# lppllppl920/SAGE-SLAM

Hardware: AMD Instinct MI355X
Metric: M residuals/sec (+ LM iters/sec), 64-keyframe feature-metric BA @128x160 (higher is better)
Workload: dtype f32; 1 GPU; 64-keyframe window, 128x160x16 feature pyramids (L=4), 32-dim depth code, dense sampling N=16128, 186 links = 372 photometric + 372 geometric directed edges; parallelism=single GPU, collective=none, accepted_steps=988

## Files before the change

include/sage_ba.h:

```cpp
#ifndef SAGE_BA_H_
#define SAGE_BA_H_

#include <stddef.h>
#include <stdint.h>

#ifdef __cplusplus
extern "C" {
#endif

#define SAGE_MAX_LEVELS 8
#define SAGE_POSE_FLOATS 12

#define SAGE_OK 0
#define SAGE_E_INVALID (-1)
#define SAGE_E_UNSUPPORTED (-2)
#define SAGE_E_NOT_PSD (-3)
#define SAGE_E_STATE (-4)
#define SAGE_E_NO_OVERLAP (-5)

typedef struct SageCamera
{
  float fx, fy, cx, cy, w, h;
} SageCamera;

// ... 10 lines not shown
const char *sage_version(void);
const char *sage_error_string(int code);

typedef struct SageWorkspace SageWorkspace;
int sage_workspace_create(void *hip_stream, SageWorkspace **out);
void sage_workspace_destroy(SageWorkspace *ws);


int sage_photometric_jac_error_calculate(
    SageWorkspace *ws, float *AtA_dev, float *Atb_dev, float *error_host, float *num_inliers_host,
    const float *R10_dev, const float *t10_dev, const float *R0_dev, const float *t0_dev,
    const float *R1_dev, const float *t1_dev,
    const float *bias0_dev, const float *basis0_dev, const float *code0_dev, const float *mask1_dev,
    const int64_t *loc1d_dev, const float *homo_dev,
    const float *feat0_dev, const float *feat1_dev, const float *grad1_dev,
    float scale0, const SagePyramid *pyr, float eps, const float *weights_host,
    int N, int FS, int CS);

int sage_photometric_error_calculate(
    SageWorkspace *ws, float *error_host, float *num_inliers_host,
    const float *R10_dev, const float *t10_dev,
    const float *bias0_dev, const float *basis0_dev, const float *code0_dev, const float *mask1_dev,
    const int64_t *loc1d_dev, const float *homo_dev,
    const float *feat0_dev, const float *feat1_dev,
    float scale0, const SagePyramid *pyr, float eps, const float *weights_host,
    int N, int FS, int CS);

int sage_tracker_photo_jac_error_calculate(
    SageWorkspace *ws, int dof, float *AtA_dev, float *Atb_dev, float *error_host, float *num_inliers_host,
    const float *R_dev, const float *t_dev, const float *mask1_dev,
    const float *dpts0_dev, const float *homo_dev, const float *feat0s_dev,
    const float *feat1_dev, const float *grad1_dev,
    const SagePyramid *pyr, float scale0, float eps, const float *weights_dev, int N, int FS);

int sage_tracker_photo_error_calculate(
    SageWorkspace *ws, float *error_host, float *num_inliers_host,
    const float *R_dev, const float *t_dev, const float *mask1_dev,
    const float *dpts0_dev, const float *homo_dev, const float *feat0s_dev, const float *feat1_dev,
    const SagePyramid *pyr, float eps, const float *weights_dev, int N, int FS);

int sage_geometric_jac_error_calculate(
    SageWorkspace *ws, float *AtA_dev, float *Atb_dev, float *error_host, float *num_inliers_host,
    const float *R10_dev, const float *t10_dev, const float *R0_dev, const float *t0_dev,
    const float *R1_dev, const float *t1_dev,
    const float *bias0_dev, const float *basis0_dev, const float *code0_dev,
    const float *dpt1_dev, const float *dpt_grad1_dev, const float *basis1_dev, const float *mask1_dev,
    const int32_t *loc1d_dev, const float *homo_dev,
    float scale0, float scale1, const SageCamera *cam, float eps, float loss_param, float weight,
    int N, int CS);

int sage_geometric_error_calculate(
    SageWorkspace *ws, float *error_host, float *num_inliers_host,
    const float *R10_dev, const float *t10_dev,
    const float *bias0_dev, const float *basis0_dev, const float *code0_dev,
    const float *dpt1_dev, const float *mask1_dev, const int32_t *loc1d_dev, const float *homo_dev,
    float scale0, const SageCamera *cam, float eps, float loss_param, float weight, int N, int CS);

int sage_depth_and_grad(SageWorkspace *ws, float *dpt_dev, float *dpt_grad_dev,
                        const float *bias_dev, const float *basis_dev, const float *code_dev,
                        float scale, int H, int W, int CS);
int sage_gaussian_pyramid_with_grad(SageWorkspace *ws, float *pyr_dev, float *grad_dev,
                                    const float *feat_dev, const float *mask_dev,
                                    const SagePyramid *pyr, int FS);

int sage_bind_thread_to_device(int device);
int sage_solver_helper_cpus(int *cpus, int n);
int sage_solver_placement_moves(void);
int sage_placement_monitor(int enable);
void sage_shutdown(void);
int sage_host_threads_running(void);

void sage_se3_exp(const float *omega, const float *v, float *R, float *t);
void sage_pose_retract(const float *pose, const float *delta6, float *out);
int sage_nearest_psd(const double *M, int n, double *out);
int sage_nearest_psd_reference(const double *M, int n, double *out);
int sage_factor_block_count(int type, int CS);
int sage_factor_hessian_blocks(int type, int CS, const float *AtA_host, const float *Atb_host, int psd_mode,
                               double *G_out, double *g_out, int32_t *dims_out, int32_t *nkeys_out);
int sage_damped_solve_qr_f32(const float *A, const float *b, int n, float damp, float *x);

int sage_block_solve(const double *packed_host, int K, int nlinks, const int32_t *links, int B, double damp,
                     const double *diag_add, const double *g_add, double *delta);
long long sage_solve_lookahead_count(void);

typedef struct SageLmConfig
{
  int max_num_iters;
  float min_grad_thresh;
  float min_param_inc_thresh;
  float init_damp;
  float min_damp, max_damp;
  float damp_dec_factor;
  float damp_inc_factor;
  float jac_update_err_inc_threshold;
  int max_inner_evals;
  float no_overlap_error;
  int linearize_at_candidate;
} SageLmConfig;
void sage_lm_config_default(SageLmConfig *cfg);

typedef int (*SageTrackLinearizeFn)(void *ctx, const float *pose12, float scale, float *AtA, float *Atb, float *error);
typedef int (*SageTrackErrorFn)(void *ctx, const float *pose12, float scale, float *error);

typedef struct SageLmTraceEntry
{
  float damp, error, candidate_error;
  int accepted, relinearized;
} SageLmTraceEntry;

int sage_track_lm(const SageLmConfig *cfg, int dof, SageTrackLinearizeFn lin, SageTrackErrorFn err, void *ctx,
                  float *pose12, float *scale, float *final_error, int *iters,
                  SageLmTraceEntry *trace, int trace_cap, int *trace_len);

typedef struct SageTrackProblem
{
  SageWorkspace *ws;
  int32_t use_photo;
  const float *mask1_dev, *dpts0_dev, *homo_dev, *feat0s_dev, *feat1_dev, *grad1_dev;
  const float *weights_dev;
  SagePyramid pyr;
  float eps;
  int32_t N, FS;
  int32_t use_keypoints, NK;
  const float *kp_dpts0_dev;
  const float *kp_homo0_dev;
  const float *kp_matched_2d_dev;
  const float *kp_matched_dpts1_dev;
  const float *kp_matched_homo1_dev;
  float kp_loss_param;
  float kp_weight;
} SageTrackProblem;
int sage_track_frame(const SageLmConfig *cfg, int dof, const SageTrackProblem *prob,
                     float *pose12, float *scale, float *final_error, int *iters,
                     SageLmTraceEntry *trace, int trace_cap, int *trace_len);

typedef struct SageOverlapStats
{
  double input_area, warp_area;
  float area_ratio, inlier_ratio, average_motion;
  int32_t n_points, n_pos_depth, n_in_mask;
  int32_t n_candidates[2];
} SageOverlapStats;
int sage_track_overlap(SageWorkspace *ws, const float *R, const float *t, const float *dpts0_dev, float depth_scale,
                       const float *homo_dev, int M, const SageCamera *cam, const float *mask_dev, float eps,
                       SageOverlapStats *out);
int sage_convex_hull_area(const float *xy, int n, double *area, int *n_vertices);

typedef struct SageWindow SageWindow;

typedef struct SageKeyframeView
{
  const float *feat_pyr;
  const float *grad_pyr;
  const float *bias;
  const float *basis;
  const int64_t *loc1d;
  const float *homo;
  int32_t N;
} SageKeyframeView;

typedef struct SageWindowConfig
{
  SagePyramid pyr;
  int32_t FS, CS;
  const float *mask_dev;
  float photo_weights[SAGE_MAX_LEVELS];
// ... 105 lines not shown
                                        const float *matched_2d, const SageCamera *cam, float eps, float loss_param,
                                        float weight, int N);

enum { SAGE_LOSS_FAIR = 0, SAGE_LOSS_L2 = 1, SAGE_LOSS_HUBER = 2, SAGE_LOSS_UNBIASED = 3 };
int sage_match_geometry_jac_error_calculate(SageWorkspace *ws, float *AtA_dev, float *Atb_dev, float *error_host,
                                            const float *R10, const float *t10, const float *R0, const float *t0,
                                            const float *R1, const float *t1, const float *bias0, const float *bias1,
                                            const float *basis0, const float *basis1, const float *code0,
                                            const float *code1, const float *homo0, const float *matched_homo1,
                                            const int32_t *loc1d_0, const int32_t *matched_loc1d_1, float scale0,
                                            float scale1, float loss_param, float weight, int loss, int N, int CS);
int sage_match_geometry_error_calculate(SageWorkspace *ws, float *error_host, const float *R10, const float *t10,
                                        const float *bias0, const float *bias1, const float *basis0, const float *basis1,
                                        const float *code0, const float *code1, const float *homo0,
                                        const float *matched_homo1, const int32_t *loc1d_0,
                                        const int32_t *matched_loc1d_1, float scale0, float scale1, float loss_param,
                                        float weight, int loss, int N, int CS);
int sage_loop_mg_jac_error_calculate(SageWorkspace *ws, float *AtA_dev, float *Atb_dev, float *error_host,
                                     const float *R10, const float *t10, const float *R0, const float *t0,
                                     const float *R1, const float *t1, const float *unscaled_dpts0,
                                     const float *matched_unscaled_dpts1, const float *homo0, const float *matched_homo1,
                                     float scale0, float scale1, float loss_param, float weight, int N);
int sage_loop_mg_error_calculate(SageWorkspace *ws, float *error_host, const float *R10, const float *t10,
                                 const float *unscaled_dpts0, const float *matched_unscaled_dpts1, const float *homo0,
                                 const float *matched_homo1, float scale0, float scale1, float loss_param, float weight,
                                 int N);
int sage_tracker_match_geom_jac_error_calculate(SageWorkspace *ws, float *AtA_dev, float *Atb_dev, float *error_host,
                                                const float *R, const float *t, const float *sampled_dpts0,
                                                const float *matched_dpts1, const float *homo0,
                                                const float *matched_homo1, float scale0, float loss_param,
                                                float weight, int with_scale, int N);
int sage_tracker_match_geom_error_calculate(SageWorkspace *ws, float *error_host, const float *R, const float *t,
                                            const float *sampled_dpts0, const float *matched_dpts1, const float *homo0,
                                            const float *matched_homo1, float loss_param, float weight, int N);

int sage_cycle_match(SageWorkspace *ws, const float *desc0_dev, const float *desc1_dev, const int64_t *kp_loc1d_0,
                     int K, int C, int H, int W, float cyc_thresh, int64_t *raw_matched_loc1d_1,
                     int64_t *cyc_matched_loc1d_0, int32_t *inlier_flags, int *n_inliers_host);

int sage_sort_locations(SageWorkspace *ws, const int64_t *loc1d_dev, const float *homo_dev, int n, int H, int W,
                        int64_t *loc1d_out_dev, float *homo_out_dev, int *sorted_host);
int sage_valid_locations(SageWorkspace *ws, const float *mask_dev, const SageCamera *cam, int64_t *loc1d_dev,
                         float *homo_dev, int *n_valid_host);
int sage_shuffle_indices(int64_t seed, int64_t n, int64_t *idx_host);
int sage_sample_locations(SageWorkspace *ws, const int64_t *valid_loc1d_dev, const float *valid_homo_dev, int n_valid,
                          int64_t seed, int num_samples, int64_t *loc1d_dev, float *homo_dev, int *n_out_host);

typedef int (*SageAllReduceFn)(double *dev_buf, size_t n, void *user);
int sage_window_set_allreduce(SageWindow *w, SageAllReduceFn fn, void *user);

typedef struct SageShardPlan SageShardPlan;
int sage_shard_plan_create(int K, int nlinks, const int32_t *links, int B, int rank, int world, SageShardPlan **out);
void sage_shard_plan_destroy(SageShardPlan *p);
size_t sage_shard_sep_count(const SageShardPlan *p);
int sage_shard_num_separators(const SageShardPlan *p);
int sage_shard_num_interior(const SageShardPlan *p);
int sage_shard_keyframe_owner(const SageShardPlan *p, int kf);
int sage_shard_keyframe_is_local(const SageShardPlan *p, int kf);
int sage_shard_eliminate(SageShardPlan *p, const double *packed_local_host, double damp, const double *diag_add,
                         const double *g_add, double *sep_out);
int sage_shard_solve(SageShardPlan *p, const double *sep_reduced, double *delta);
int sage_shard_plan_create_domains(int K, int nlinks, const int32_t *links, int B, int domain, int ndomains,
                                   SageShardPlan **out);
int sage_block_solve_domains(const double *packed_host, int K, int nlinks, const int32_t *links, int B, double damp,
                             const double *diag_add, const double *g_add, int ndomains, double *delta);

int sage_window_emulate_peers(SageWindow *w, const double *rest_dev, int n_iterates);
#define SAGE_RCCL_ID_BYTES 128
int sage_rccl_unique_id(unsigned char *id128);
int sage_rccl_comm_create(const unsigned char *id128, int rank, int world, void **comm_out);
void sage_rccl_comm_destroy(void *comm);
int sage_rccl_comm_info(void *comm, int *ranks_out, int *rank_out);
int sage_window_use_rccl(SageWindow *w, void *nccl_comm);

typedef struct SageLmState
{
  double damp, error, candidate_error;
  int accepted, iters;
} SageLmState;
int sage_window_lm_step(SageWindow *w, SageLmState *st, const SageLmConfig *cfg);
int sage_window_lm_run(SageWindow *w, SageLmState *st, const SageLmConfig *cfg, int n, double *trace, int *done);
int sage_window_lm_run_timed(SageWindow *w, SageLmState *st, const SageLmConfig *cfg, int n, double *trace, int *done,
                             double *step_seconds);
int sage_window_sync_variables(SageWindow *w);

#ifdef __cplusplus
}
#endif
#endif
```

sage_slam_amd/build.py:

```python
from __future__ import annotations

import os
import subprocess
import sys
from concurrent.futures import ThreadPoolExecutor

HERE = os.path.dirname(os.path.abspath(__file__))
ROOT = os.path.dirname(HERE)
CSRC = os.path.join(HERE, "csrc")
OBJ = os.path.join(HERE, "csrc", "_obj")
LIB = os.path.join(HERE, "libsage_ba.so")
SOURCES = ["photo_kernels.hip", "geo_kernels.hip", "track_kernels.hip", "producers.hip", "keypoint_kernels.hip", "graph_kernels.hip", "solve_kernels.hip", "operators.hip", "tracker.hip", "overlap.hip", "window.hip", "window_eval.hip", "window_reduce.hip", "window_solve.hip", "window_lm.hip", "window_profile.hip", "window_build.hip", "window_terms.hip", "window_dist.hip", "window_factors.hip",
           "host_math.cpp", "block_solver.cpp", "host_threads.cpp", "shard_solve.cpp", "convex_hull.cpp"]
HEADERS = ["sage_device.h", "sage_internal.h", "damped_system.h", "host_math.h", "block_solver.h", "host_threads.h", "runtime_internal.h", "window_state.h", "finalize_bodies.h", "keypoint_batch.h", "graph_terms.h", "graph_batch.h", "term_results.h", "window_plan.h", os.path.join(ROOT, "include", "sage_ba.h")]
HIPCC = os.environ.get("HIPCC", "/opt/rocm/bin/hipcc")
HOSTCXX = os.environ.get("HOSTCXX", "/opt/rocm/lib/llvm/bin/clang++")
FLAGS = ["--offload-arch=gfx950", "-O3", "-std=c++17", "-fPIC", "-Wall", "-Wno-unused-function",
         "-I" + os.path.join(ROOT, "include"), "-I" + CSRC]


def kernel_source_sha16() -> str:
    import hashlib
    h = hashlib.sha256()
    for f in ("photo_kernels.hip", "geo_kernels.hip", "sage_device.h", "sage_internal.h"):
        with open(os.path.join(CSRC, f), "rb") as fh:
            h.update(fh.read())
    return h.hexdigest()[:16]


def _mtime(p):
    return os.path.getmtime(p) if os.path.exists(p) else 0.0


def _compile(src):
    obj = os.path.join(OBJ, os.path.splitext(src)[0] + ".o")
    deps = [os.path.join(CSRC, src)] + [h if os.path.isabs(h) else os.path.join(CSRC, h) for h in HEADERS]
    if _mtime(obj) >= max(_mtime(d) for d in deps):
        return obj, False
    if src.endswith(".hip"):
        cmd = [HIPCC] + FLAGS + ["-x", "hip", "-c", os.path.join(CSRC, src), "-o", obj]
    else:
        cmd = [HOSTCXX, "-O3", "-std=c++17", "-fPIC", "-Wall", "-I" + os.path.join(ROOT, "include"), "-I" + CSRC,
               "-c", os.path.join(CSRC, src), "-o", obj]
    subprocess.check_call(cmd)
    return obj, True


def build(force: bool = False, verbose: bool = False) -> str:
    os.makedirs(OBJ, exist_ok=True)
    if force:
        for f in os.listdir(OBJ):
            os.remove(os.path.join(OBJ, f))
    with ThreadPoolExecutor(max_workers=min(8, len(SOURCES))) as ex:
        res = list(ex.map(_compile, SOURCES))
    objs = [o for o, _ in res]
    if any(ch for _, ch in res) or not os.path.exists(LIB):
        subprocess.check_call([HIPCC, "--offload-arch=gfx950", "-shared", "-fPIC", "-o", LIB] + objs + ["-lpthread"])
        if verbose:
            print("built", LIB)
    return LIB


GLUE_SRC = os.path.join(ROOT, "integration", "compile_check", "prepass_run.cpp")
GLUE_BIN = os.path.join(ROOT, "integration", "compile_check", "_bin", "prepass_run")
REF_THIRDPARTY = "/root/reference/system/thirdparty"


def build_glue_check(verbose: bool = False):
    if not os.path.isdir(REF_THIRDPARTY):
        return GLUE_BIN if os.path.exists(GLUE_BIN) else None
    deps = [GLUE_SRC, os.path.join(ROOT, "integration", "sage_gtsam_prepass.h"), os.path.join(ROOT, "include", "sage_ba.h"),
            os.path.join(ROOT, "integration", "compile_check", "gtsam", "linear", "HessianFactor.h"),
            os.path.join(ROOT, "integration", "compile_check", "gtsam", "nonlinear", "Values.h"), LIB]
    if _mtime(GLUE_BIN) >= max(_mtime(d) for d in deps):
        return GLUE_BIN
    os.makedirs(os.path.dirname(GLUE_BIN), exist_ok=True)
    subprocess.check_call([HOSTCXX, "-std=c++17", "-O1", "-w", "-D__HIP_PLATFORM_AMD__", "-I" + os.path.join(ROOT, "include"),
                           "-I" + os.path.join(ROOT, "integration", "compile_check"), "-I" + REF_THIRDPARTY + "/eigen",
                           "-I" + REF_THIRDPARTY + "/Sophus", "-I/opt/rocm/include", GLUE_SRC, "-o", GLUE_BIN,
                           "-L" + HERE, "-lsage_ba", "-L/opt/rocm/lib", "-lamdhip64",
                           "-Wl,-rpath,$ORIGIN/../../../sage_slam_amd", "-Wl,-rpath,/opt/rocm/lib"])
    if verbose:
        print("built", GLUE_BIN)
    return GLUE_BIN


ADAPTER_BIN = os.path.join(ROOT, "integration", "compile_check", "_bin", "adapter_run")
REF_SYSTEM = "/root/reference/system"


def build_adapter_run(verbose: bool = False):
    if not os.path.isdir(REF_SYSTEM):
        return ADAPTER_BIN if os.path.exists(ADAPTER_BIN) else None
    import torch
    T = os.path.dirname(torch.__file__)
    srcs = [os.path.join(ROOT, "integration", "sage_adapter.cpp"), os.path.join(ROOT, "integration", "sage_adapter_keypoints.cpp"),
            os.path.join(ROOT, "integration", "compile_check", "adapter_run.cpp")]
# ... 31 lines not shown
```

sage_slam_amd/capi.py:

```python
from __future__ import annotations

import ctypes as C
import os
from typing import List, Optional, Sequence

import numpy as np

HERE = os.path.dirname(os.path.abspath(__file__))
LIB_PATH = os.path.join(HERE, "libsage_ba.so")
SAGE_MAX_LEVELS = 8


class SageError(RuntimeError):
    def __init__(self, code: int, where: str):
        self.code = code
        msg = lib().sage_error_string(code).decode() if _lib is not None else "?"
        super().__init__(f"{where}: {msg} (code {code})")


class SageCamera(C.Structure):
    _fields_ = [(n, C.c_float) for n in ("fx", "fy", "cx", "cy", "w", "h")]


class SagePyramid(C.Structure):
# ... 18 lines not shown
    _fields_ = [("ws", C.c_void_p), ("use_photo", C.c_int32), ("mask1_dev", C.c_void_p), ("dpts0_dev", C.c_void_p),
                ("homo_dev", C.c_void_p), ("feat0s_dev", C.c_void_p), ("feat1_dev", C.c_void_p),
                ("grad1_dev", C.c_void_p), ("weights_dev", C.c_void_p), ("pyr", SagePyramid), ("eps", C.c_float),
                ("N", C.c_int32), ("FS", C.c_int32), ("use_keypoints", C.c_int32), ("NK", C.c_int32),
                ("kp_dpts0_dev", C.c_void_p), ("kp_homo0_dev", C.c_void_p), ("kp_matched_2d_dev", C.c_void_p),
                ("kp_matched_dpts1_dev", C.c_void_p), ("kp_matched_homo1_dev", C.c_void_p),
                ("kp_loss_param", C.c_float), ("kp_weight", C.c_float)]


class SageKeyframeView(C.Structure):
    _fields_ = [("feat_pyr", C.c_void_p), ("grad_pyr", C.c_void_p), ("bias", C.c_void_p), ("basis", C.c_void_p),
                ("loc1d", C.c_void_p), ("homo", C.c_void_p), ("N", C.c_int32)]


class SageWindowConfig(C.Structure):
    _fields_ = [("pyr", SagePyramid), ("FS", C.c_int32), ("CS", C.c_int32), ("mask_dev", C.c_void_p),
                ("photo_weights", C.c_float * SAGE_MAX_LEVELS), ("geo_weight", C.c_float),
                ("geo_loss_param", C.c_float), ("eps", C.c_float), ("code_prior_weight", C.c_float),
                ("scale_prior_weight", C.c_float), ("pose_prior_weight", C.c_float),
                ("use_photo", C.c_int32), ("use_geo", C.c_int32)]


SAGE_KP_REPROJECTION, SAGE_KP_MATCH_GEOMETRY, SAGE_KP_LOOP_MG = 0, 1, 2
SAGE_HOLD_POSE, SAGE_HOLD_CODE, SAGE_HOLD_SCALE = 1, 2, 4
KP_KINDS = {"reprojection": SAGE_KP_REPROJECTION, "match_geometry": SAGE_KP_MATCH_GEOMETRY, "loop_mg": SAGE_KP_LOOP_MG}


class SageKeypointTerm(C.Structure):
    _fields_ = [("kind", C.c_int32), ("edge", C.c_int32), ("N", C.c_int32), ("loc1d_0", C.c_void_p), ("homo0", C.c_void_p),
                ("matched_2d", C.c_void_p), ("matched_loc1d_1", C.c_void_p), ("matched_homo1", C.c_void_p),
                ("loss_param", C.c_float), ("weight", C.c_float), ("loss", C.c_int32), ("unscaled_dpts0", C.c_void_p),
                ("matched_unscaled_dpts1", C.c_void_p)]


def kp_term_dim(kind, CS: int) -> int:
    kind = KP_KINDS.get(kind, kind)
    return {SAGE_KP_REPROJECTION: 13 + CS, SAGE_KP_MATCH_GEOMETRY: 14 + 2 * CS, SAGE_KP_LOOP_MG: 14}[kind]


SAGE_GRAPH_REL_POSE_SCALE, SAGE_GRAPH_REL_POSE, SAGE_GRAPH_SCALE_PRIOR = 0, 1, 2
GRAPH_KINDS = {"rel_pose_scale": SAGE_GRAPH_REL_POSE_SCALE, "rel_pose": SAGE_GRAPH_REL_POSE, "scale_prior": SAGE_GRAPH_SCALE_PRIOR}
GRAPH_TERM_DIM = 14
GRAPH_KIND_ROWS = {SAGE_GRAPH_REL_POSE_SCALE: 7, SAGE_GRAPH_REL_POSE: 6, SAGE_GRAPH_SCALE_PRIOR: 1}


class SageGraphTerm(C.Structure):
    _fields_ = [("kind", C.c_int32), ("edge", C.c_int32), ("kf", C.c_int32), ("target_pose10", C.c_float * 12),
                ("target_scale0", C.c_float), ("target_scale1", C.c_float), ("weight", C.c_float), ("rot_weight", C.c_float),
                ("scale_weight", C.c_float)]


def graph_term_struct(t) -> SageGraphTerm:
    gt = SageGraphTerm()
    gt.kind = int(GRAPH_KINDS.get(t["kind"], t["kind"]))
    gt.edge, gt.kf = int(t.get("edge", 0)), int(t.get("kf", 0))
    tp = np.asarray(t.get("target_pose10", [1, 0, 0, 0, 1, 0, 0, 0, 1, 0, 0, 0]), np.float32).reshape(12)
    for i in range(12):
        gt.target_pose10[i] = float(tp[i])
    gt.target_scale0, gt.target_scale1 = float(t.get("target_scale0", 1.0)), float(t.get("target_scale1", 1.0))
    gt.weight, gt.rot_weight, gt.scale_weight = float(t["weight"]), float(t.get("rot_weight", 1.0)), float(t.get("scale_weight", 1.0))
    return gt


ALLREDUCE_FN = C.CFUNCTYPE(C.c_int, C.c_void_p, C.c_size_t, C.c_void_p)


class SageLmState(C.Structure):
    _fields_ = [("damp", C.c_double), ("error", C.c_double), ("candidate_error", C.c_double),
                ("accepted", C.c_int), ("iters", C.c_int)]


TRACK_LIN_FN = C.CFUNCTYPE(C.c_int, C.c_void_p, C.POINTER(C.c_float), C.c_float, C.POINTER(C.c_float),
                           C.POINTER(C.c_float), C.POINTER(C.c_float))
TRACK_ERR_FN = C.CFUNCTYPE(C.c_int, C.c_void_p, C.POINTER(C.c_float), C.c_float, C.POINTER(C.c_float))

_lib = None

SYMBOLS = [
    "sage_camera_pyramid", "sage_version", "sage_error_string", "sage_workspace_create", "sage_workspace_destroy",
    "sage_photometric_jac_error_calculate", "sage_photometric_error_calculate",
    "sage_tracker_photo_jac_error_calculate", "sage_tracker_photo_error_calculate",
    "sage_geometric_jac_error_calculate", "sage_geometric_error_calculate", "sage_depth_and_grad",
    "sage_gaussian_pyramid_with_grad", "sage_se3_exp", "sage_pose_retract", "sage_nearest_psd", "sage_nearest_psd_reference", "sage_factor_block_count", "sage_factor_hessian_blocks",
    "sage_damped_solve_qr_f32", "sage_block_solve", "sage_solve_lookahead_count", "sage_lm_config_default", "sage_track_lm", "sage_track_frame", "sage_track_overlap", "sage_convex_hull_area",
    "sage_window_create", "sage_window_destroy", "sage_window_add_keyframe", "sage_window_add_link", "sage_window_add_keypoint_link", "sage_window_hold", "sage_window_set_link_geo_loss",
    "sage_window_set_shard", "sage_window_finalize", "sage_window_num_keyframes", "sage_window_num_links",
    "sage_window_block_size", "sage_window_solver_block_size", "sage_window_packed_count", "sage_window_packed_dev",
    "sage_window_residuals_per_linearize", "sage_window_bytes_per_linearize", "sage_window_linearize",
    "sage_window_error", "sage_window_tune_runs", "sage_window_set_runs", "sage_window_error_dev", "sage_window_solve", "sage_window_total_error",
    "sage_window_accept", "sage_window_reset", "sage_window_get_keyframe", "sage_window_set_keyframe", "sage_window_get_delta",
    "sage_window_get_edge", "sage_window_add_keypoint_term", "sage_window_num_keypoint_terms", "sage_window_get_keypoint_term", "sage_window_add_graph_term", "sage_window_num_graph_terms", "sage_window_get_graph_term", "sage_window_prepass", "sage_window_factor", "sage_window_factor_error", "sage_window_prepare_factors", "sage_factor_psd", "sage_factor_cut_blocks", "sage_window_set_profiling", "sage_window_get_kernel_time", "sage_window_get_phase_time", "sage_window_lm_step", "sage_window_lm_run", "sage_window_lm_run_timed", "sage_window_sync_variables", "sage_window_set_allreduce", "sage_shard_plan_create", "sage_shard_plan_create_domains", "sage_block_solve_domains", "sage_shard_plan_destroy", "sage_shard_sep_count", "sage_shard_num_separators", "sage_shard_num_interior", "sage_shard_keyframe_owner", "sage_shard_keyframe_is_local", "sage_shard_eliminate", "sage_shard_solve", "sage_rccl_unique_id", "sage_rccl_comm_create", "sage_rccl_comm_destroy", "sage_rccl_comm_info", "sage_window_use_rccl", "sage_window_emulate_peers", "sage_sort_locations", "sage_bind_thread_to_device", "sage_solver_helper_cpus", "sage_solver_placement_moves", "sage_placement_monitor", "sage_shutdown", "sage_host_threads_running",
    "sage_valid_locations", "sage_shuffle_indices", "sage_sample_locations",
    "sage_reprojection_jac_error_calculate", "sage_reprojection_error_calculate",
    "sage_tracker_reproj_jac_error_calculate", "sage_tracker_reproj_error_calculate",
    "sage_match_geometry_jac_error_calculate", "sage_match_geometry_error_calculate",
    "sage_loop_mg_jac_error_calculate", "sage_loop_mg_error_calculate",
    "sage_tracker_match_geom_jac_error_calculate", "sage_tracker_match_geom_error_calculate", "sage_cycle_match",
]


def lib():
    global _lib
    if _lib is None:
        LIB_PATH = os.environ.get("SAGE_BA_LIB", globals()["LIB_PATH"])
        if not os.path.exists(LIB_PATH):
            raise ImportError(f"{LIB_PATH} is missing: run `python -m sage_slam_amd.build` "
                              "(the HIP engine has no fallback path)")
        import torch
        L = C.CDLL(LIB_PATH)
        L.sage_version.restype = C.c_char_p
        L.sage_error_string.restype = C.c_char_p
        L.sage_window_packed_count.restype = C.c_size_t
        L.sage_shutdown.restype = None
        L.sage_window_packed_dev.restype = C.c_void_p
        L.sage_window_error_dev.restype = C.c_void_p
        L.sage_window_residuals_per_linearize.restype = C.c_double
        L.sage_window_bytes_per_linearize.restype = C.c_double
        for name in ("sage_window_packed_count", "sage_window_packed_dev", "sage_window_error_dev",
                     "sage_window_residuals_per_linearize", "sage_window_bytes_per_linearize",
                     "sage_window_num_keyframes", "sage_window_num_links", "sage_window_block_size",
                     "sage_window_solver_block_size"):
            getattr(L, name).argtypes = [C.c_void_p]
        _lib = L
    return _lib


def _chk(code: int, where: str):
    if code != 0:
        raise SageError(code, where)


def _f32(a) -> np.ndarray:
    return np.ascontiguousarray(a, dtype=np.float32)


def _fp(a: np.ndarray):
    return a.ctypes.data_as(C.POINTER(C.c_float))


def dptr(t) -> C.c_void_p:
    if t is None:
        return C.c_void_p(0)
    assert t.is_contiguous(), "device buffers handed to the C ABI must be contiguous"
    return C.c_void_p(t.data_ptr())


def make_pyramid(cam, levels: int) -> SagePyramid:
    base = SageCamera(*[float(v) for v in (cam.fx, cam.fy, cam.cx, cam.cy, cam.w, cam.h)])
    out = SagePyramid()
    _chk(lib().sage_camera_pyramid(C.byref(base), levels, C.byref(out)), "sage_camera_pyramid")
    return out


def se3_exp(omega, v):
    omega = _f32(omega); v = _f32(v)
    R = np.zeros(9, np.float32); t = np.zeros(3, np.float32)
    lib().sage_se3_exp(_fp(omega), _fp(v), _fp(R), _fp(t))
    return R.reshape(3, 3), t


def pose_retract(pose12, delta6):
    pose12 = _f32(pose12).reshape(12); delta6 = _f32(delta6)
    out = np.zeros(12, np.float32)
    lib().sage_pose_retract(_fp(pose12), _fp(delta6), _fp(out))
    return out


def nearest_psd(M):
    M = np.ascontiguousarray(M, dtype=np.float64)
    out = np.zeros_like(M)
    _chk(lib().sage_nearest_psd(M.ctypes.data_as(C.POINTER(C.c_double)), M.shape[0],
                                out.ctypes.data_as(C.POINTER(C.c_double))), "sage_nearest_psd")
    return out


def nearest_psd_reference(M):
    M = np.ascontiguousarray(M, np.float64)
    out = np.zeros_like(M)
    _chk(lib().sage_nearest_psd_reference(M.ctypes.data_as(C.POINTER(C.c_double)), M.shape[0],
                                          out.ctypes.data_as(C.POINTER(C.c_double))), "sage_nearest_psd_reference")
    return out


def factor_hessian_blocks(type_: int, CS: int, AtA, Atb, psd_mode: int = 1):
    L = lib()
    A = _f32(AtA); b = _f32(Atb)
    n = L.sage_factor_block_count(type_, CS)
    if n < 0:
        raise SageError(n, "sage_factor_block_count")
    G = np.zeros(n, np.float64); g = np.zeros(b.size, np.float64)
    dims = (C.c_int32 * 6)(); nk = C.c_int32()
    _chk(L.sage_factor_hessian_blocks(type_, CS, _fp(A), _fp(b), psd_mode, G.ctypes.data_as(C.POINTER(C.c_double)),
                                      g.ctypes.data_as(C.POINTER(C.c_double)), dims, C.byref(nk)),
         "sage_factor_hessian_blocks")
    dims = [int(dims[i]) for i in range(nk.value)]
    blocks, o = {}, 0
    for i in range(nk.value):
        for j in range(i, nk.value):
            blocks[(i, j)] = G[o:o + dims[i] * dims[j]].reshape(dims[i], dims[j]); o += dims[i] * dims[j]
    offs = np.concatenate([[0], np.cumsum(dims)])
    return blocks, [g[offs[i]:offs[i + 1]] for i in range(nk.value)], dims


def damped_solve_qr_f32(A, b, damp):
    A = _f32(A); b = _f32(b)
    x = np.zeros(b.shape[0], np.float32)
    _chk(lib().sage_damped_solve_qr_f32(_fp(A), _fp(b), b.shape[0], C.c_float(damp), _fp(x)), "sage_damped_solve_qr_f32")
    return x


def block_solve(packed, K, links, B, damp, diag_add=None, g_add=None):
    packed = np.ascontiguousarray(packed, dtype=np.float64)
    lk = np.ascontiguousarray(np.asarray(links, dtype=np.int32).reshape(-1))
    delta = np.zeros(K * B, np.float64)
    dp = lambda a: None if a is None else np.ascontiguousarray(a, np.float64).ctypes.data_as(C.POINTER(C.c_double))
    da = None if diag_add is None else np.ascontiguousarray(diag_add, np.float64)
    ga = None if g_add is None else np.ascontiguousarray(g_add, np.float64)
    _chk(lib().sage_block_solve(packed.ctypes.data_as(C.POINTER(C.c_double)), K, len(lk) // 2, lk.ctypes.data_as(C.POINTER(C.c_int32)), B,
                                C.c_double(damp), dp(da), dp(ga), delta.ctypes.data_as(C.POINTER(C.c_double))),
         "sage_block_solve")
    return delta


def solve_lookahead_count() -> int:
    f = lib().sage_solve_lookahead_count
    f.restype = C.c_longlong
    return int(f())


def block_solve_domains(packed, K, links, B, damp, ndomains, diag_add=None, g_add=None):
    p = np.ascontiguousarray(packed, np.float64)
    lk = np.ascontiguousarray(np.asarray(links, np.int32).reshape(-1))
    out = np.zeros(K * B, np.float64)
    dp = lambda a: None if a is None else np.ascontiguousarray(a, np.float64).ctypes.data_as(C.POINTER(C.c_double))
    da = None if diag_add is None else np.ascontiguousarray(diag_add, np.float64)
    ga = None if g_add is None else np.ascontiguousarray(g_add, np.float64)
    _chk(lib().sage_block_solve_domains(p.ctypes.data_as(C.POINTER(C.c_double)), K, len(links),
                                        lk.ctypes.data_as(C.POINTER(C.c_int32)), B, C.c_double(damp), dp(da), dp(ga),
                                        ndomains, out.ctypes.data_as(C.POINTER(C.c_double))), "sage_block_solve_domains")
    return out


def lm_config_default() -> SageLmConfig:
    cfg = SageLmConfig()
    lib().sage_lm_config_default(C.byref(cfg))
    return cfg


def pack_pose(R, t) -> np.ndarray:
    return np.concatenate([_f32(R).reshape(9), _f32(t).reshape(3)])


def track_lm(cfg: SageLmConfig, dof: int, lin_fn, err_fn, pose12, scale: float, trace_cap: int = 256):
    def _lin(ctx, p, s, AtA, Atb, err):
        A, b, e = lin_fn(np.ctypeslib.as_array(p, (12,)).copy(), float(s))
        A = _f32(A).reshape(-1); b = _f32(b).reshape(-1)
        for i in range(dof * dof):
            AtA[i] = A[i]
        for i in range(dof):
            Atb[i] = b[i]
        err[0] = e
        return 0

    def _err(ctx, p, s, err):
        err[0] = err_fn(np.ctypeslib.as_array(p, (12,)).copy(), float(s))
        return 0

    pose = _f32(pose12).reshape(12).copy()
    sc = C.c_float(scale)
    fe = C.c_float(0); it = C.c_int(0); tl = C.c_int(0)
    trace = (SageLmTraceEntry * trace_cap)()
    cb1, cb2 = TRACK_LIN_FN(_lin), TRACK_ERR_FN(_err)
    _chk(lib().sage_track_lm(C.byref(cfg), dof, cb1, cb2, None, _fp(pose), C.byref(sc), C.byref(fe), C.byref(it),
                             trace, trace_cap, C.byref(tl)), "sage_track_lm")
    tr = [dict(damp=trace[i].damp, error=trace[i].error, candidate_error=trace[i].candidate_error,
               accepted=trace[i].accepted, relinearized=trace[i].relinearized) for i in range(tl.value)]
    return pose, sc.value, fe.value, it.value, tr


def track_frame(cfg: SageLmConfig, dof: int, prob: "SageTrackProblem", pose12, scale: float, trace_cap: int = 256):
    L = lib()
    p = _f32(pose12).copy()
    sc = C.c_float(scale); fe = C.c_float(); it = C.c_int(); tl = C.c_int()
    tr = (SageLmTraceEntry * trace_cap)()
    rc = L.sage_track_frame(C.byref(cfg), dof, C.byref(prob), _fp(p), C.byref(sc), C.byref(fe), C.byref(it), tr,
                            trace_cap, C.byref(tl))
    trace = [dict(damp=tr[i].damp, error=tr[i].error, candidate_error=tr[i].candidate_error,
                  accepted=tr[i].accepted, relinearized=tr[i].relinearized) for i in range(tl.value)]
    return rc, p, sc.value, fe.value, it.value, trace


class SageOverlapStats(C.Structure):
    _fields_ = [("input_area", C.c_double), ("warp_area", C.c_double), ("area_ratio", C.c_float),
                ("inlier_ratio", C.c_float), ("average_motion", C.c_float), ("n_points", C.c_int32),
                ("n_pos_depth", C.c_int32), ("n_in_mask", C.c_int32), ("n_candidates", C.c_int32 * 2)]


def track_overlap_raw(ws_handle, R, t, dpts0_ptr, depth_scale, homo_ptr, M, cam_ptr, mask_ptr, eps, out_ptr) -> int:
    f = lib().sage_track_overlap
    f.argtypes = [C.c_void_p, C.c_void_p, C.c_void_p, C.c_void_p, C.c_float, C.c_void_p, C.c_int, C.c_void_p, C.c_void_p,
                  C.c_float, C.c_void_p]
    return int(f(ws_handle, R, t, dpts0_ptr, depth_scale, homo_ptr, int(M), cam_ptr, mask_ptr, eps, out_ptr))


# ... 320 lines not shown
        return out

    def packed_tensor(self):
        return _tensor_from_ptr(lib().sage_window_packed_dev(self.h), self.packed_count)

    def error_tensor(self):
        return _tensor_from_ptr(lib().sage_window_error_dev(self.h), 4)

    def linearize(self):
        _chk(lib().sage_window_linearize(self.h), "sage_window_linearize")

    def error(self, which=1):
        _chk(lib().sage_window_error(self.h, which), "sage_window_error")

    def tune_runs(self):
        tpb, rule = C.c_int(0), C.c_int(0)
        ms_rule, ms_best = C.c_float(0), C.c_float(0)
        _chk(lib().sage_window_tune_runs(self.h, C.byref(tpb), C.byref(rule), C.byref(ms_rule), C.byref(ms_best)),
             "sage_window_tune_runs")
        return dict(tpb=tpb.value, tpb_rule=rule.value, ms_rule=ms_rule.value, ms_best=ms_best.value)

    def set_runs(self, tpb):
        _chk(lib().sage_window_set_runs(self.h, int(tpb)), "sage_window_set_runs")

    def solve(self, damp, want_norm=True):
        if not want_norm:
            _chk(lib().sage_window_solve(self.h, C.c_double(damp), None), "sage_window_solve")
            return None
        sn = C.c_double()
        _chk(lib().sage_window_solve(self.h, C.c_double(damp), C.byref(sn)), "sage_window_solve")
        return sn.value

    def total_error(self, from_linearize: bool):
        e = C.c_double()
        _chk(lib().sage_window_total_error(self.h, int(from_linearize), C.byref(e)), "sage_window_total_error")
        return e.value

    def accept(self):
        _chk(lib().sage_window_accept(self.h), "sage_window_accept")

    def reset(self):
        _chk(lib().sage_window_reset(self.h), "sage_window_reset")

    def set_allreduce(self, dist_module, group=None):
        tensors = {}
        for t in (self.packed_tensor(), self.error_tensor()):
            tensors[(t.data_ptr(), t.numel())] = t

        def hook(ptr, n, _user):
            try:
                t = tensors.get((ptr, n))
                if t is None:
                    t = tensors[(ptr, n)] = _tensor_from_ptr(ptr, n)
                dist_module.all_reduce(t, group=group)
                return 0
            except Exception:
                import traceback
                traceback.print_exc()
                return 1

        self._allreduce_cb = ALLREDUCE_FN(hook)
        _chk(lib().sage_window_set_allreduce(self.h, self._allreduce_cb, None), "sage_window_set_allreduce")

    def sync_variables(self):
        _chk(lib().sage_window_sync_variables(self.h), "sage_window_sync_variables")

    def use_rccl(self, comm):
        _chk(lib().sage_window_use_rccl(self.h, C.c_void_p(comm)), "sage_window_use_rccl")

    def emulate_peers(self, rest):
        if rest is None:
            self._emu_rest = None
            _chk(lib().sage_window_emulate_peers(self.h, None, 0), "sage_window_emulate_peers")
            return
        assert rest.is_cuda and rest.dim() == 2 and rest.shape[1] == self.packed_count and rest.is_contiguous()
        self._emu_rest = rest
        _chk(lib().sage_window_emulate_peers(self.h, C.c_void_p(rest.data_ptr()), int(rest.shape[0])),
             "sage_window_emulate_peers")

    def lm_step(self, state: SageLmState, cfg: SageLmConfig):
        _chk(lib().sage_window_lm_step(self.h, C.byref(state), C.byref(cfg)), "sage_window_lm_step")
        return state

    def lm_run(self, state: SageLmState, cfg: SageLmConfig, n: int):
        tr = np.zeros((n, 4), np.float64)
        done = C.c_int()
        _chk(lib().sage_window_lm_run(self.h, C.byref(state), C.byref(cfg), n, tr.ctypes.data_as(C.POINTER(C.c_double)),
                                      C.byref(done)), "sage_window_lm_run")
        return tr[:done.value]

    def lm_run_timed(self, state: SageLmState, cfg: SageLmConfig, n: int):
        tr = np.zeros((n, 4), np.float64); sec = np.zeros(n, np.float64)
        done = C.c_int()
        _chk(lib().sage_window_lm_run_timed(self.h, C.byref(state), C.byref(cfg), n, tr.ctypes.data_as(C.POINTER(C.c_double)),
                                            C.byref(done), sec.ctypes.data_as(C.POINTER(C.c_double))), "sage_window_lm_run_timed")
        return tr[:done.value], sec[:done.value]

    def delta(self):
        d = np.zeros(self.K * self.B, np.float64)
        _chk(lib().sage_window_get_delta(self.h, d.ctypes.data_as(C.POINTER(C.c_double))), "sage_window_get_delta")
        return d

    def get_keyframe(self, k):
        pose = np.zeros(12, np.float32); code = np.zeros(self.win.CS, np.float32); s = C.c_float()
        _chk(lib().sage_window_get_keyframe(self.h, k, _fp(pose), _fp(code), C.byref(s)), "sage_window_get_keyframe")
        return pose, code, s.value

    def set_keyframe(self, k, pose12, code, scale):
        pose12 = _f32(pose12); code = _f32(code)
        _chk(lib().sage_window_set_keyframe(self.h, k, _fp(pose12), _fp(code), C.c_float(scale)),
             "sage_window_set_keyframe")

    def get_edge(self, type_, e):
        D = 13 + self.win.CS if type_ == 0 else 14 + 2 * self.win.CS
        A = np.zeros((D, D), np.float32); b = np.zeros(D, np.float32)
        err = C.c_float(); nin = C.c_float()
        _chk(lib().sage_window_get_edge(self.h, type_, e, _fp(A), _fp(b), C.byref(err), C.byref(nin)),
             "sage_window_get_edge")
        return dict(AtA=A, Atb=b, error=err.value, num_inliers=nin.value)

    def prepass(self, poses12, codes, scales, jacobians: bool = True) -> bool:
        P = _f32(np.asarray(poses12).reshape(-1)); Cd = _f32(np.asarray(codes).reshape(-1)); S = _f32(np.asarray(scales).reshape(-1))
        K = self.K
        assert P.size == K * 12 and Cd.size == K * self.win.CS and S.size == K
        rec = C.c_int32()
        _chk(lib().sage_window_prepass(self.h, _fp(P), _fp(Cd), _fp(S), int(jacobians), C.byref(rec)), "sage_window_prepass")
        return bool(rec.value)

    def factor(self, type_, e, psd_mode: int = 1):
        L = lib(); CS = self.win.CS
        n = L.sage_factor_block_count(type_, CS)
        D = 13 + CS if type_ == 0 else 14 + 2 * CS
        G = np.zeros(n, np.float64); g = np.zeros(D, np.float64); f = C.c_double()
        dims = (C.c_int32 * 6)(); nk = C.c_int32()
        _chk(L.sage_window_factor(self.h, type_, e, psd_mode, G.ctypes.data_as(C.POINTER(C.c_double)),
                                  g.ctypes.data_as(C.POINTER(C.c_double)), C.byref(f), dims, C.byref(nk)), "sage_window_factor")
        dims = [int(dims[i]) for i in range(nk.value)]
        blocks, o = {}, 0
        for i in range(nk.value):
            for j in range(i, nk.value):
                blocks[(i, j)] = G[o:o + dims[i] * dims[j]].reshape(dims[i], dims[j]); o += dims[i] * dims[j]
        offs = np.concatenate([[0], np.cumsum(dims)])
        return blocks, [g[offs[i]:offs[i + 1]] for i in range(nk.value)], f.value, dims

    def prepare_factors(self, psd_mode: int = 1, n_threads: int = 0):
        _chk(lib().sage_window_prepare_factors(self.h, psd_mode, n_threads), "sage_window_prepare_factors")

    def factor_error(self, type_, e) -> float:
        v = C.c_double()
        _chk(lib().sage_window_factor_error(self.h, type_, e, C.byref(v)), "sage_window_factor_error")
        return v.value

    def set_profiling(self, on):
        _chk(lib().sage_window_set_profiling(self.h, int(on)), "sage_window_set_profiling")

    def kernel_time(self, which: int):
        ms = C.c_double(); n = C.c_int()
        _chk(lib().sage_window_get_kernel_time(self.h, which, C.byref(ms), C.byref(n)), "sage_window_get_kernel_time")
        return ms.value, n.value

    def phase_time(self):
        ms = (C.c_double * 4)(); n = C.c_int()
        _chk(lib().sage_window_get_phase_time(self.h, ms, C.byref(n)), "sage_window_get_phase_time")
        return dict(zip(("linearize", "allreduce", "solve", "error_pass"), (float(v) for v in ms))), n.value

    def packed_host(self):
# ... 366 lines not shown
```

sage_slam_amd/csrc/block_solver.cpp:

```cpp
#include <algorithm>
#include <atomic>
#include <chrono>
#include <cmath>
#include <cstdio>
#include <cstdlib>
#include <cstring>
#include <sched.h>
#include <thread>
#include <vector>

#include "block_solver.h"
#include "damped_system.h"
#include "host_math.h"
#include "sage_ba.h"

namespace sage
{
namespace
{
typedef double v8d __attribute__((vector_size(64), aligned(8)));

#define SAGE_LOADU(dst, p) __builtin_memcpy(&(dst), (p), sizeof(v8d))
#define SAGE_STOREU(p, v) __builtin_memcpy((p), &(v), sizeof(v8d))

// ... 1498 lines not shown
  {
    const int rc = block_chol_range(E0, T, X, y, 0, K);
    return rc ? rc : block_back_range(E0, T, X, y, 0, K);
  }
  const int sep0 = E0.n1 + E0.n2;
  BlockEnvelope E = E0;
  const bool arrow = block_plan_has_arrow_rows(E0);
  SepJob job;
  SepPool *pool = nullptr;
  if (arrow)
  {
    job.E = &E; job.T = T; job.X = X; job.y = y;
    sep_job_build(job);
    job.t_start = mono_seconds();
    E.progress = job.progress;
    pool = pool_engage(job);
  }
  BlockEnvelope::RowPipe pipes[2];
  E.pipe = pipes;
  static const bool no_sep_pre = sage::env_flag("SAGE_SOLVE_NO_SEP_PRE");
  E.sep_pre = !arrow && !no_sep_pre;
  CholHelper *h = helper_engage(E, T, X, y);
  const bool piped = lookahead_engage(1, E, T, X, y, 0, E.n1);
  const bool dbg = debug_timing();
  double tp[6] = {0, 0, 0, 0, 0, 0};
  auto lap = [&](int k) {
    if (dbg)
      tp[k] = mono_seconds();
  };
  lap(0);
  int rc = block_chol_range(E, T, X, y, 0, E.n1, piped ? RowRole::chain : RowRole::whole);
  if (piped)
    lookahead_release(1);
  lap(1);
  const bool helper_has_it = h && helper_claimed(h);
  const int rc2 = helper_has_it ? helper_join_factor(h) : rc == 0 ? block_chol_range(E, T, X, y, E.n1, sep0) : 0;
  lap(2);
  if (rc == 0)
    rc = rc2;
  if (arrow)
    rc = arrow_separator(job, rc, tp[2]);
  else if (rc == 0)
    rc = block_chol_range(E, T, X, y, sep0, K);
  if (rc == 0)
    block_back_range(E, T, X, y, sep0, K);
  if (arrow)
  {
    arrow_back_substitute(job, E, rc);
    if (pool)
      pool_release(pool);
  }
  lap(3);
  if (helper_has_it)
    helper_go_back(h, rc == 0);
  if (rc == 0)
  {
    block_back_range(E, T, X, y, 0, E.n1);
    if (!helper_has_it)
      block_back_range(E, T, X, y, E.n1, sep0);
  }
  lap(4);
  if (helper_has_it)
    helper_join_back(h);
  lap(5);
  if (dbg)
    fprintf(stderr, "[sage block chol] us: first half %.0f (+wait for the %s %.0f) separator %.0f%s back-subst %.0f (+wait %.0f)\n",
            1e6 * (tp[1] - tp[0]), helper_has_it ? "helper" : "second half, same thread", 1e6 * (tp[2] - tp[1]),
            1e6 * (tp[3] - tp[2]), arrow ? (pool ? " (arrow rows, worker pool)" : " (arrow rows, no pool)") : "",
            1e6 * (tp[4] - tp[3]), 1e6 * (tp[5] - tp[4]));
  if (h)
    helper_release(h);
  return rc;
}

BlockEnvelope envelope_of(const BlockPlan &plan, int Bp)
{
  BlockEnvelope env;
  env.K = (int)plan.row_first.size(); env.Bp = Bp; env.n1 = plan.n1; env.n2 = plan.n2;
  env.row_first = plan.row_first.data(); env.row_off = plan.row_off.data();
  env.a_first = plan.a_first.data(); env.a_cnt = plan.a_cnt.data(); env.a_off = plan.a_off.data();
  env.col_ptr = plan.col_ptr.data(); env.col_rows = plan.col_rows.data();
  return env;
}
}

extern "C" long long sage_solve_lookahead_count(void) { return sage::g_lookahead_count.load(); }

extern "C" int sage_block_solve(const double *packed, int K, int nlinks, const int32_t *links, int B, double damp,
                                const double *diag_add, const double *g_add, double *delta)
{
  if (!packed || K < 1 || B < 1 || nlinks < 0 || (nlinks > 0 && !links) || !delta)
    return SAGE_E_INVALID;
  const int Bp = sage::padded_block(B);
  if (Bp == 0)
    return SAGE_E_UNSUPPORTED;
  const int BB = B * B, BBp = Bp * Bp;
  const double *diag = packed;
  const double *lnk = diag + (size_t)K * BB;
  const double *g = lnk + (size_t)nlinks * BB;
  std::vector<std::pair<int, int>> lk(nlinks);
  for (int l = 0; l < nlinks; ++l)
    lk[l] = {links[2 * l], links[2 * l + 1]};
  sage::BlockPlan bp;
  int rcp = sage::plan_blocks(K, lk, !sage::env_flag("SAGE_SOLVE_NO_SPLIT"), bp);
  if (rcp == SAGE_E_UNSUPPORTED)
  {
    std::sort(lk.begin(), lk.end());
    lk.erase(std::unique(lk.begin(), lk.end()), lk.end());
    rcp = sage::plan_blocks(K, lk, !sage::env_flag("SAGE_SOLVE_NO_SPLIT"), bp);
  }
  if (rcp != SAGE_OK)
    return rcp;
  const int nblk = bp.nblk;
  std::vector<double> T((size_t)nblk * BBp, 0.0), X((size_t)K * BBp), y((size_t)K * Bp, 0.0);
  for (int q = 0; q < K; ++q)
  {
    const int k = bp.perm[q];
    double *D = T.data() + (size_t)bp.index(q, q) * BBp;
    for (int r = 0; r < Bp; ++r)
      for (int c = 0; c < Bp; ++c)
        D[sage::stored_slot(r, c, Bp)] =
            (r < B && c < B) ? sage::damped_diag_elem(diag + (size_t)k * BB, B, r, c, diag_add ? diag_add[k * B + r] : 0.0, damp)
                             : sage::damped_pad_elem(r, c, damp);
    for (int r = 0; r < B; ++r)
      y[(size_t)q * Bp + r] = sage::damped_rhs_elem(g[(size_t)k * B + r], g_add ? g_add[k * B + r] : 0.0);
  }
  for (int l = 0; l < nlinks; ++l)
  {
    const int a = links[2 * l], b = links[2 * l + 1];
    const int qi = std::max(bp.pos[a], bp.pos[b]), qj = std::min(bp.pos[a], bp.pos[b]);
    double *D = T.data() + (size_t)bp.index(qi, qj) * BBp;
    const bool row_is_a = bp.perm[qi] == a;
    for (int r = 0; r < B; ++r)
      for (int c = 0; c < B; ++c)
        D[sage::stored_slot(r, c, Bp)] += lnk[(size_t)l * BB + sage::link_elem(row_is_a, r, c, B)];
  }
  static const bool dbg = sage::env_flag("SAGE_DEBUG_TIMING");
  const auto t0 = std::chrono::steady_clock::now();
  sage::BlockEnvelope env = sage::envelope_of(bp, Bp);
  int rcf;
  {
    sage::SolveLease lease;
    if (bp.n1 > 0)
      env.no_lookahead = sage::block_chol_arm(sage::block_plan_has_arrow_rows(env), sage::block_plan_long_arrow_chains(env));
    rcf = sage::block_chol_solve_tr(env, T.data(), X.data(), y.data());
  }
  if (dbg)
    fprintf(stderr, "[sage block_solve] fixed-block Cholesky + substitution %.3f ms\n",
            std::chrono::duration<double, std::milli>(std::chrono::steady_clock::now() - t0).count());
  if (rcf != 0)
    return SAGE_E_NOT_PSD;
  for (int k = 0; k < K; ++k)
    std::memcpy(delta + (size_t)k * B, y.data() + (size_t)bp.pos[k] * Bp, sizeof(double) * B);
  return SAGE_OK;
}
```

sage_slam_amd/csrc/block_solver.h:

```cpp
#pragma once
#include <stdint.h>

#include <algorithm>
#include <atomic>
#include <utility>
#include <vector>

#include "host_threads.h"

namespace sage
{
inline int padded_block(int B) { return B < 1 ? 0 : B <= 8 ? 8 : B <= 24 ? 24 : B <= 40 ? 40 : 0; }

struct BlockEnvelope
{
  int K = 0, Bp = 0;
  const int32_t *row_first = nullptr, *row_off = nullptr;
  const int32_t *a_first = nullptr, *a_cnt = nullptr, *a_off = nullptr;
  int n1 = 0, n2 = 0;
  const volatile unsigned *ready = nullptr;
  unsigned epoch = 0;
  const uint8_t *fill = nullptr;
  bool no_lookahead = false;
  std::atomic<int> *progress = nullptr;
  const int32_t *col_ptr = nullptr, *col_rows = nullptr;
  int bs_skip_from = 0x7fffffff;
  struct RowPipe
  {
    alignas(64) std::atomic<int> early{0};
    alignas(64) std::atomic<int> late{0};
    alignas(64) std::atomic<int> pre{0};
  };
  RowPipe *pipe = nullptr;
  bool sep_pre = false;

  struct Range
  {
    int lo, hi;
  };
  Range a_range(int i) const
  {
    const int a = a_cnt ? a_first[i] : 0;
    return {a, a + (a_cnt ? a_cnt[i] : 0)};
  }
  Range b_range(int i) const { return {row_first[i], i}; }
  bool has(int i, int j) const
  {
    const Range a = a_range(i);
    return (j >= row_first[i] && j <= i) || (j >= a.lo && j < a.hi);
  }
  size_t index(int i, int j) const
  {
    return (size_t)(j < row_first[i] ? a_off[i] + j - a_first[i] : row_off[i] + j - row_first[i]);
  }
  double *block(double *T, int i, int j) const { return T + index(i, j) * (size_t)(Bp * Bp); }
  Range sep_range(int srow, int half) const
  {
    if (half == 0)
      return a_range(srow);
    const int sep0 = n1 + n2;
    return {std::min((int)row_first[srow], sep0), sep0};
  }
};
int block_chol_solve_tr(const BlockEnvelope &env, double *T, double *X, double *y);
int block_chol_partial(const BlockEnvelope &env, double *T, double *X, double *y, int nI);
int block_chol_partial_back(const BlockEnvelope &env, double *T, double *X, double *y, int nI);
int block_plan_long_arrow_chains(const BlockEnvelope &env);
bool block_plan_has_arrow_rows(const BlockEnvelope &env);

struct BlockPlan
{
  std::vector<int32_t> perm, pos, row_first, row_off, a_first, a_cnt, a_off, blk_row, blk_col, blk_src;
  std::vector<int32_t> col_ptr, col_rows;
  int nblk = 0, n1 = 0, n2 = 0;
  int index(int i, int j) const
  {
    return j < row_first[i] ? a_off[i] + j - a_first[i] : row_off[i] + j - row_first[i];
  }
};
int plan_blocks(int K, const std::vector<std::pair<int, int>> &links, bool may_split, BlockPlan &out);
BlockEnvelope envelope_of(const BlockPlan &plan, int Bp);
}
```

sage_slam_amd/csrc/runtime_internal.h:

```cpp
#pragma once

#include <hip/hip_runtime.h>

#include <algorithm>
#include <atomic>
#include <cctype>
#include <sched.h>
#include <chrono>
#include <cmath>
#include <cstdlib>
#include <cstdio>
#include <cstring>
#include <thread>
#include <vector>

#include <dlfcn.h>
#if __has_include(<rccl/rccl.h>)
#include <rccl/rccl.h>
#else
extern "C"
{
  typedef struct ncclComm *ncclComm_t;
  typedef struct
  {
    char internal[128];
  } ncclUniqueId;
  typedef enum { ncclSuccess = 0 } ncclResult_t;
  typedef enum { ncclSum = 0 } ncclRedOp_t;
  typedef enum { ncclDouble = 8 } ncclDataType_t;
}
#endif

#include "host_math.h"
#include "host_threads.h"
#include "sage_ba.h"
#include "sage_internal.h"
#include "keypoint_batch.h"
#include "graph_batch.h"
#include "window_plan.h"

using namespace sage;

#define SAGE_HIP(expr)                \
  do                                  \
  {                                   \
    hipError_t _e = (expr);           \
    if (_e != hipSuccess)             \
      return (int)_e;                 \
  } while (0)

namespace sage_rt
{

struct DevBuf
{
  void *p = nullptr;
  size_t cap = 0;
  DevBuf() = default;
  DevBuf(const DevBuf &) = delete;
  DevBuf &operator=(const DevBuf &) = delete;
  DevBuf(DevBuf &&o) noexcept { swap(o); }
  DevBuf &operator=(DevBuf &&o) noexcept
  {
    DevBuf(std::move(o)).swap(*this);
    return *this;
  }
  ~DevBuf() { release(); }
  void swap(DevBuf &o) noexcept
  {
    std::swap(p, o.p);
    std::swap(cap, o.cap);
  }
  int reserve(size_t bytes)
  {
    if (bytes <= cap)
      return 0;
    release();
    hipError_t e = hipMalloc(&p, bytes);
    if (e != hipSuccess)
    {
      p = nullptr;
      return (int)e;
    }
    cap = bytes;
    return 0;
  }
  void release()
  {
    if (p)
      (void)hipFree(p);
    p = nullptr;
    cap = 0;
  }
  template <class T>
  T *as() const { return reinterpret_cast<T *>(p); }
};

inline int pick_tiles_per_block(long long total_tiles)
{
  if (total_tiles >= 8192)
    return 4;
  if (total_tiles >= 4096)
    return 2;
  return 1;
}

struct WorkList
{
  std::vector<WorkItem> work;
  std::vector<int32_t> edge_first, edge_tiles;
  std::vector<int32_t> rec_first, rec_count;
  int tiles_per_block = 1;
  int flush = 1;
  int n_records = 0;
  void build(const std::vector<int> &N, int tpb_override = 0, const std::vector<int> *order = nullptr, int flush_ = 0)
  {
    long long total = 0;
    for (int n : N)
      total += (n + kTile - 1) / kTile;
// ... 48 lines not shown
static inline bool supported(int CS, int FS)
{
  return (CS == 16 || CS == 32) && (FS == 16 || FS == 32);
}

namespace sage
{
struct AdjEntry
{
  int32_t type;
  int32_t edge;
  int32_t role;
};

struct LinkEdges
{
  int32_t e_ab, e_ba;
};

struct AssembleParams
{
  const float *AtA_p, *Atb_p, *stats_p;
  const float *AtA_g, *Atb_g, *stats_g;
  const double *wide_p, *wide_g;
  const int32_t *adj_start;
  const AdjEntry *adj;
  const LinkEdges *links;
  double *packed;
  double *tail_mirror;
  int K, nlinks, CS, n_edges_p, n_edges_g;
  int split;
  const int32_t *blocks;
  const int32_t *link_terms_start;
  const AdjEntry *link_terms;
  TermResults terms;
};

struct ErrorTotalsSide
{
  const int32_t *edge_first, *edge_tiles;
  const float *partials;
  float *stats;
  float fallback, scale;
  int n_edges;
  int stride, err_off, cnt_off;
};

}

#include "window_state.h"

struct SageWindow
{
  SageWindowConfig cfg;
  hipStream_t stream = nullptr;
  bool finalized = false;
  int rank = 0, world = 1;
  int K = 0, B = 0, VS = 0;
  std::vector<SageKeyframeView> views;
  HostVars hv;
  std::vector<float> link_geo_loss;
  std::vector<std::pair<int, int>> links;
  std::vector<char> link_dense;
  std::vector<uint8_t> hold;
  sage::plan::SolverRows rows;
  std::vector<int> local_links;
  std::vector<int> owned_edges;
  std::vector<int> local_edges;
  int n_edges = 0;
  DevBuf vars[2];
  DevBuf sorted_loc, sorted_homo;
  std::vector<std::pair<const int64_t *, const float *>> user_samples;
  std::vector<int> user_n;
  DevBuf dpt, dgrad, depth_items[2];
  int n_depth = 0;
  int dpt_set = -1;
  bool dgrad_valid = false;
  DevBuf geo_px;
  bool merge_ok = false;
  DevBuf pk;
  DevBuf f0s;
  DenseSide dense[2];
  PhotoRecordPlan photo_rec;
  std::vector<int> Nedge;
  int tpb_heur = 1;
  DevBuf adj_start, adj, link_edges, packed, errbuf;
  TotalsMirror mirror;
  WindowDist dist;
  std::vector<double> host_packed;
  std::vector<double> delta;
  sage::DeviceSolver *solver = nullptr;
  bool cand_pending = false;
  double residuals_per_lin = 0, bytes_per_lin = 0;
  bool have_lin = false;
  uint64_t vars_epoch = 1, lin_epoch = 0;
  bool spec_err_valid = false;
  double spec_error = 0.0;
  DevBuf packed_save;
  TermSide terms;
  struct FactorCache
  {
    bool lin = false, err = false;
    std::vector<float> pose, code, scale;
    struct Side
    {
      std::vector<float> A, b, s;
      std::vector<double> C;
    } side[2];
    int psd_mode = -1;
  } fc;
  WindowProfiler prof;

  bool kernels_mirror_totals() const { return world == 1 && !dist.allreduce && mirror.h; }
};


template <class T>
static int upload(DevBuf &b, const std::vector<T> &v, hipStream_t s)
{
  int rc = b.reserve(std::max<size_t>(v.size(), 1) * sizeof(T));
  if (rc)
    return rc;
  if (!v.empty())
    SAGE_HIP(hipMemcpyAsync(b.p, v.data(), v.size() * sizeof(T), hipMemcpyHostToDevice, s));
  return 0;
}
int window_upload_vars(SageWindow *w, int set);
int window_local_edge(const SageWindow *w, int global_edge);
bool window_owns_edge(const SageWindow *w, int global_edge);
bool window_has_holds(const SageWindow *w);
std::vector<int32_t> window_link_pairs(const SageWindow *w);
struct FinalizeState
{
  bool domain_solve = false;
  std::vector<char> needed;
  std::vector<size_t> f0s_off;
  std::vector<size_t> px_off;
  std::vector<int> Nedge;
  std::vector<std::vector<AdjEntry>> adjv;
  std::vector<LinkEdges> le;
  std::vector<char> link_terms;
  double residuals = 0, bytes = 0;
};
int finalize_terms(SageWindow *w, FinalizeState &fs);
int window_launch_terms(SageWindow *w, int set, bool jac);
int window_linearize_set(SageWindow *w, int set, double *dst = nullptr, bool local_blocks = false, bool merge = false);
int window_error_pass(SageWindow *w, int which, bool speculate_gradients);
int window_collective(SageWindow *w, double *buf, size_t n);
int window_allreduce(SageWindow *w, double *buf, size_t n, int iterate);
int window_allreduce_into(SageWindow *w, const double *send, double *recv, size_t n, int iterate);
int window_mirror_totals(SageWindow *w, bool with_err, const double *system = nullptr);
bool window_wait_error_totals(SageWindow *w);
bool window_wait_reduced_totals(SageWindow *w);
int window_wait_mirror(SageWindow *w, bool *not_psd);
double mirrored_error(const SageWindow *w, int at, int set);
int window_total_error(SageWindow *w, int from_linearize, double *err, bool stream_idle);
int window_copy_floats(SageWindow *w, const float *src, float *dst, int n);
void window_add_to_double(SageWindow *w, double *p, double v);
double window_prior_error(const SageWindow *w, int set, bool owned_only = false);
int window_sync_candidate(SageWindow *w, bool stream_idle = false);
int window_schur_solve(SageWindow *w, double damp, double *lin_error);
void prof_attach(SageWindow *w, int which, LaunchCommon &lc);
void window_phase_mark(SageWindow *w, int which);
```

sage_slam_amd/csrc/solve_kernels.hip:

```cpp
#include <algorithm>
#include <atomic>
#include <chrono>
#include <cstdio>
#include <cstring>
#include <memory>
#include <vector>

#include "block_solver.h"
#include "damped_system.h"
#include "host_math.h"
#include "sage_device.h"
#include "sage_internal.h"
#include "window_plan.h"

namespace sage
{

struct SolvePlan
{
  int K, B, Bs, Bp, nblk, nlinks;
  const int32_t *row_first;
  const int32_t *row_off;
  const int32_t *blk_row, *blk_col, *blk_src;
  const int32_t *perm, *pos;
  const int32_t *hold;
  const int32_t *to_block, *to_solver;
};

struct SolveResult
{
  double step_norm2;
  int status;
  unsigned go;
};
static size_t result_vars_offset() { return sizeof(SolveResult); }
static size_t result_delta_offset(int K, int VS) { return (sizeof(SolveResult) + (size_t)K * VS * sizeof(float) + 15) / 16 * 16; }

constexpr int kScatterWorkgroups = 32;

__global__ __launch_bounds__(256) void solve_scatter_kernel(const SolvePlan P, const double *__restrict__ packed,
                                                            const float *__restrict__ vars0, int VS, int CS,
                                                            const SolvePriors pri, double damp,
                                                            double *__restrict__ L, double *__restrict__ y,
                                                            const int32_t *__restrict__ order, unsigned *flags,
                                                            unsigned epoch)
{
  const int tid = threadIdx.x;
  const int B = P.B, Bs = P.Bs, Bp = P.Bp, BB = B * B;
  __shared__ double s_dadd[64], s_gadd[64];
  __shared__ int s_row[64];
  if (tid < Bs)
    s_row[tid] = P.to_block[tid];
  __syncthreads();
  for (int it = blockIdx.x; it < P.nblk; it += gridDim.x)
  {
    const int b = order[it];
    const int i = P.blk_row[b], j = P.blk_col[b], srcf = P.blk_src[b];
    const int src = srcf < 0 ? -1 : (srcf & 0x3fffffff);
    const bool row_is_a = srcf >= 0 && (srcf & 0x40000000);
    if (src < 0 && i != j)
      continue;
    const int kf = P.perm[i];
    const int hold_r = P.hold ? P.hold[kf] : 0, hold_c = P.hold ? P.hold[P.perm[j]] : 0;
    const double *diag = packed + (size_t)kf * BB;
    const double *lnk = packed + (size_t)P.K * BB + (size_t)(src < 0 ? 0 : src) * BB;
    const double *g = packed + (size_t)P.K * BB + (size_t)P.nlinks * BB + (size_t)kf * B;
    double *out = L + (size_t)b * Bp * Bp;
    if (i == j)
    {
      const float *var = vars0 + (size_t)kf * VS;
      if (tid < Bs)
      {
        double da, ga;
        prior_row(pri, kf, s_row[tid], CS, var, var[12], var + 13, da, ga, hold_r);
        s_dadd[tid] = da;
        s_gadd[tid] = ga;
      }
      __syncthreads();
    }
    for (int o = tid; o < Bp * Bp; o += blockDim.x)
    {
      const int c = o / Bp, r = o - c * Bp;
      double v = 0.0;
      const bool in = r < Bs && c < Bs;
      const bool held = in && solver_elem_held(hold_r, hold_c, s_row, r, c, CS);
      if (i == j)
        v = in ? (held ? held_diag_elem(r, c) : solver_diag_elem(diag, B, s_row, r, c, s_dadd[r], damp))
               : damped_pad_elem(r, c, damp);
      else if (in && !held)
        v = lnk[solver_link_elem(row_is_a, s_row, r, c, B)];
      out[o] = v;
    }
    if (i == j)
      for (int r = tid; r < Bp; r += blockDim.x)
        y[(size_t)i * Bp + r] =
            (r < Bs && !(hold_r && row_held(hold_r, s_row[r], CS))) ? damped_rhs_elem(g[s_row[r]], s_gadd[r]) : 0.0;
    __syncthreads();
    if (tid == 0)
    {
      __threadfence_system();
      *reinterpret_cast<volatile unsigned *>(flags + b) = epoch;
    }
  }
}

__global__ __launch_bounds__(1024) void solve_retract_kernel(const double *__restrict__ x, int K, int B, int Bp, int CS,
                                                            int VS, const int32_t *__restrict__ pos,
                                                            const int32_t *__restrict__ hold,
                                                            const int32_t *__restrict__ to_solver,
                                                            const float *__restrict__ vars0,
                                                            float *__restrict__ vars1, float *__restrict__ h_vars,
                                                            double *__restrict__ h_delta, SolveResult *h_res,
                                                            unsigned epoch)
{
  const int tid = threadIdx.x;
  const volatile unsigned *go = &h_res->go;
  __shared__ int s_go;
  if (tid == 0)
  {
    const unsigned long long t0 = wall_clock64();
    unsigned v;
    bool timed_out = false;
    for (;;)
    {
      v = *go;
      const unsigned d = ((v & 0x7fffffffu) - epoch) & 0x7fffffffu;
      if (d == 0u)
        break;
      if (d < 0x40000000u && (v & 0x7fffffffu) != 0u)
      {
        v = 0x80000000u;
        break;
      }
      __builtin_amdgcn_s_sleep(4);
      if (wall_clock64() - t0 > 200000000ull)
      {
        v = 0x80000000u;
// ... 26 lines not shown
      h_vars[(size_t)k * VS + slot] = v;
    }
  }
  for (int k = tid; k < K; k += blockDim.x)
  {
    const double *xk = x + (size_t)pos[k] * Bp;
    const float *v0 = vars0 + (size_t)k * VS;
    float *o = vars1 + (size_t)k * VS;
    if (hold && (hold[k] & kHoldPose))
      for (int i = 0; i < 12; ++i)
        o[i] = v0[i];
    else
    {
      float d6[6];
      for (int i = 0; i < 6; ++i)
        d6[i] = (float)xk[to_solver[i]];
      pose_retract(v0, d6, o);
    }
    for (int i = 0; i < 12; ++i)
      h_vars[(size_t)k * VS + i] = o[i];
  }
  __shared__ double s_n[16];
  for (int off = 32; off > 0; off >>= 1)
    nrm += __shfl_down(nrm, off);
  if ((tid & 63) == 0)
    s_n[tid >> 6] = nrm;
  __syncthreads();
  if (tid == 0)
  {
    double tot = 0.0;
    for (int w = 0; w < (int)(blockDim.x >> 6); ++w)
      tot += s_n[w];
    h_res->step_norm2 = tot;
  }
}

struct DeviceSolver
{
  int K = 0, B = 0, Bs = 0, Bp = 0, nblk = 0, nlinks = 0, VS = 0;
  void *d_int = nullptr;
  void *d_hold = nullptr;
  void *h_pinned = nullptr;
  void *h_T = nullptr;
  double *h_y = nullptr;
  unsigned *h_flags = nullptr;
  unsigned epoch = 0, go_epoch = 0;
  SolvePlan plan{};
  const int32_t *d_order = nullptr;
  std::vector<double> h_X;
  BlockPlan host_plan;
  std::vector<uint8_t> h_fill;

  DeviceSolver() = default;
  DeviceSolver(const DeviceSolver &) = delete;
  DeviceSolver &operator=(const DeviceSolver &) = delete;
  ~DeviceSolver()
  {
    if (d_int)
      (void)hipFree(d_int);
    if (d_hold)
      (void)hipFree(d_hold);
    if (h_pinned)
      (void)hipHostFree(h_pinned);
    if (h_T)
      (void)hipHostFree(h_T);
  }
  SolveResult *result() const { return reinterpret_cast<SolveResult *>(h_pinned); }
  float *host_vars() const { return reinterpret_cast<float *>(reinterpret_cast<char *>(h_pinned) + result_vars_offset()); }
  double *host_delta() const { return reinterpret_cast<double *>(reinterpret_cast<char *>(h_pinned) + result_delta_offset(K, VS)); }
};

int solver_create(DeviceSolver **out, int K, const plan::SolverRows &rows, int VS,
                  const std::vector<std::pair<int, int>> &links, hipStream_t stream)
{
  *out = nullptr;
  const int B = rows.B, Bs = rows.Bs;
  const int Bp = sage::padded_block(Bs);
  if (Bp == 0 || K < 1)
    return SAGE_E_UNSUPPORTED;
  BlockPlan bp;
  const int rcp = plan_blocks(K, links, !sage::env_flag("SAGE_SOLVE_NO_SPLIT"), bp);
  if (rcp != SAGE_OK)
    return rcp;
  const int n1 = bp.n1, n2 = bp.n2, nblk = bp.nblk;
  const std::vector<int32_t> &perm = bp.perm, &pos = bp.pos, &row_first = bp.row_first, &row_off = bp.row_off,
                             &a_cnt = bp.a_cnt, &a_off = bp.a_off, &blk_row = bp.blk_row, &blk_col = bp.blk_col,
                             &blk_src = bp.blk_src;
  std::unique_ptr<DeviceSolver> S(new DeviceSolver);
  S->K = K; S->B = B; S->Bs = Bs; S->Bp = Bp; S->nblk = nblk; S->nlinks = (int)links.size(); S->VS = VS;
  std::vector<int32_t> all;
  auto put = [&](const std::vector<int32_t> &v) {
    const size_t off = all.size();
    all.insert(all.end(), v.begin(), v.end());
    while (all.size() % 4)
      all.push_back(0);
    return off;
  };
  const size_t o_rf = put(row_first), o_ro = put(row_off), o_br = put(blk_row), o_bc = put(blk_col),
               o_bs = put(blk_src), o_pm = put(perm), o_ps = put(pos);
  std::vector<int32_t> order;
  auto push_row = [&](int i) {
    for (int q = 0; q < a_cnt[i]; ++q)
      order.push_back(a_off[i] + q);
    for (int q = 0; q <= i - row_first[i]; ++q)
      order.push_back(row_off[i] + q);
  };
  if (n1 > 0)
  {
    for (int t = 0; t < std::max(n1, n2); ++t)
    {
      if (t < n1)
        push_row(t);
      if (t < n2)
        push_row(n1 + t);
    }
    for (int i = n1 + n2; i < K; ++i)
      push_row(i);
  }
  else
    for (int i = 0; i < K; ++i)
      push_row(i);
  const size_t o_ord = put(order);
  const size_t o_tb = put(rows.to_block), o_ts = put(rows.to_solver);
  if (hipMalloc(&S->d_int, all.size() * sizeof(int32_t)) != hipSuccess)
    return (int)hipErrorOutOfMemory;
  if (hipMemcpyAsync(S->d_int, all.data(), all.size() * sizeof(int32_t), hipMemcpyHostToDevice, stream) != hipSuccess)
    return (int)hipErrorUnknown;
  if (hipStreamSynchronize(stream) != hipSuccess)
    return (int)hipErrorUnknown;
  const size_t ty_doubles = (size_t)nblk * Bp * Bp + (size_t)K * Bp;
  if (hipHostMalloc(&S->h_T, ty_doubles * sizeof(double) + (size_t)nblk * sizeof(unsigned), hipHostMallocDefault) !=
      hipSuccess)
    return (int)hipErrorOutOfMemory;
  S->h_y = reinterpret_cast<double *>(S->h_T) + (size_t)nblk * Bp * Bp;
  S->h_flags = reinterpret_cast<unsigned *>(reinterpret_cast<double *>(S->h_T) + ty_doubles);
  std::memset(S->h_flags, 0, (size_t)nblk * sizeof(unsigned));
  S->h_X.assign((size_t)K * Bp * Bp, 0.0);
  const size_t h_bytes = result_delta_offset(K, VS) + (size_t)K * B * sizeof(double);
  if (hipHostMalloc(&S->h_pinned, h_bytes, hipHostMallocDefault) != hipSuccess)
    return (int)hipErrorOutOfMemory;
  std::memset(S->h_pinned, 0, h_bytes);
  const int32_t *base = reinterpret_cast<const int32_t *>(S->d_int);
  SolvePlan &P = S->plan;
  P.K = K; P.B = B; P.Bs = Bs; P.Bp = Bp; P.nblk = nblk; P.nlinks = (int)links.size();
  P.row_first = base + o_rf; P.row_off = base + o_ro;
  P.blk_row = base + o_br; P.blk_col = base + o_bc; P.blk_src = base + o_bs; P.perm = base + o_pm; P.pos = base + o_ps;
  P.to_block = base + o_tb; P.to_solver = base + o_ts;
  S->d_order = base + o_ord;
  S->h_fill.assign((size_t)nblk, 0);
  for (int b = 0; b < nblk; ++b)
    S->h_fill[b] = (blk_src[b] < 0 && blk_row[b] != blk_col[b]) ? 1 : 0;
  S->host_plan = std::move(bp);
  *out = S.release();
  return SAGE_OK;
}

void solver_destroy(DeviceSolver *S) { delete S; }

int solver_set_holds(DeviceSolver *S, const std::vector<uint8_t> &hold, hipStream_t stream)
{
  if ((int)hold.size() != S->K)
    return SAGE_E_INVALID;
  const std::vector<int32_t> masks(hold.begin(), hold.end());
  if (!S->d_hold && hipMalloc(&S->d_hold, masks.size() * sizeof(int32_t)) != hipSuccess)
    return (int)hipErrorOutOfMemory;
  if (hipMemcpyAsync(S->d_hold, masks.data(), masks.size() * sizeof(int32_t), hipMemcpyHostToDevice, stream) != hipSuccess ||
      hipStreamSynchronize(stream) != hipSuccess)
    return (int)hipErrorUnknown;
  S->plan.hold = reinterpret_cast<const int32_t *>(S->d_hold);
  return SAGE_OK;
}

int solver_run(DeviceSolver *S, hipStream_t stream, const double *packed_dev, const float *vars0, float *vars1,
               int CS, double damp, const SolvePriors &pri)
{
  static const bool dbgt = sage::env_flag("SAGE_DEBUG_TIMING");
  hipError_t eh;
  SolveLease lease;
  BlockEnvelope env = envelope_of(S->host_plan, S->Bp);
  if (env.n1 > 0)
    env.no_lookahead = block_chol_arm(block_plan_has_arrow_rows(env), block_plan_long_arrow_chains(env));
  S->epoch += 1;
  if (S->epoch == 0)
    S->epoch = 1;
  hipLaunchKernelGGL(solve_scatter_kernel, dim3(std::min(kScatterWorkgroups, S->nblk)), dim3(256), 0, stream, S->plan,
                     packed_dev, vars0, S->VS, CS, pri, damp, reinterpret_cast<double *>(S->h_T), S->h_y, S->d_order,
                     S->h_flags, S->epoch);
  if ((eh = hipGetLastError()) != hipSuccess)
    return (int)eh;
  volatile unsigned *go = &S->result()->go;
  S->go_epoch = (S->go_epoch + 1) & 0x7fffffffu;
  if (S->go_epoch == 0)
    S->go_epoch = 1;
  hipLaunchKernelGGL(solve_retract_kernel, dim3(1), dim3(1024), 0, stream, S->h_y, S->K, S->B, S->Bp, CS, S->VS,
                     S->plan.pos, S->plan.hold, S->plan.to_solver, vars0, vars1, S->host_vars(), S->host_delta(),
                     S->result(), S->go_epoch);
  if ((eh = hipGetLastError()) != hipSuccess)
    return (int)eh;
  struct GoGuard
  {
    volatile unsigned *go;
    unsigned word;
    ~GoGuard()
    {
      std::atomic_thread_fence(std::memory_order_release);
      *go = word;
    }
  } guard{go, S->go_epoch | 0x80000000u};
  const auto t1 = std::chrono::steady_clock::now();
  env.ready = S->h_flags; env.epoch = S->epoch;
  env.fill = S->h_fill.data();
  const int bad = block_chol_solve_tr(env, reinterpret_cast<double *>(S->h_T), S->h_X.data(), S->h_y);
  const auto t2 = std::chrono::steady_clock::now();
  if (dbgt)
    fprintf(stderr, "[sage hybrid solve] wait for the system + host cholesky %.3f ms\n",
            std::chrono::duration<double, std::milli>(t2 - t1).count());
  if (bad == -2)
    return SAGE_E_STATE;
  if (bad)
    return SAGE_E_NOT_PSD;
  guard.word = S->go_epoch;
  return SAGE_OK;
}

const float *solver_host_vars(const DeviceSolver *S) { return S->host_vars(); }
const double *solver_host_delta(const DeviceSolver *S) { return S->host_delta(); }
double solver_host_step_norm2(const DeviceSolver *S) { return S->result()->step_norm2; }
int solver_host_status(const DeviceSolver *S) { return S->result()->status; }

}
```

sage_slam_amd/csrc/window_build.hip:

```cpp
#include "runtime_internal.h"
#include "window_plan.h"

static std::atomic<int> g_live_windows{0};

extern "C" int sage_window_create(const SageWindowConfig *cfg, void *hip_stream, SageWindow **out)
{
  if (!cfg || !out || !cfg->mask_dev)
    return SAGE_E_INVALID;
  if (!supported(cfg->CS, cfg->FS) || cfg->pyr.levels < 1 || cfg->pyr.levels > SAGE_MAX_LEVELS)
    return SAGE_E_UNSUPPORTED;
  int ndev = 0;
  SAGE_HIP(hipGetDeviceCount(&ndev));
  if (ndev < 1)
    return (int)hipErrorNoDevice;
  SageWindow *w = new SageWindow();
  w->cfg = *cfg;
  w->stream = reinterpret_cast<hipStream_t>(hip_stream);
  w->B = 7 + cfg->CS;
  w->VS = ((13 + cfg->CS + 3) / 4) * 4;
  *out = w;
  g_live_windows.fetch_add(1, std::memory_order_acq_rel);
  return SAGE_OK;
}

// ... 16 lines not shown
}

extern "C" int sage_window_add_keyframe(SageWindow *w, const SageKeyframeView *v, const float *pose12,
                                        const float *code, float scale)
{
  if (!w || !v || !pose12 || !code || w->finalized)
    return SAGE_E_INVALID;
  if (!v->feat_pyr || !v->grad_pyr || !v->bias || !v->basis || !v->loc1d || !v->homo || v->N < 0)
    return SAGE_E_INVALID;
  w->views.push_back(*v);
  for (int s = 0; s < 2; ++s)
  {
    w->hv.pose[s].insert(w->hv.pose[s].end(), pose12, pose12 + 12);
    w->hv.code[s].insert(w->hv.code[s].end(), code, code + w->cfg.CS);
    w->hv.scale[s].push_back(scale);
  }
  w->hv.pose_init.insert(w->hv.pose_init.end(), pose12, pose12 + 12);
  w->hv.code_added.insert(w->hv.code_added.end(), code, code + w->cfg.CS);
  w->hv.scale_init.push_back(scale);
  return w->K++;
}

static int add_link(SageWindow *w, int a, int b, char dense)
{
  if (a == b || a < 0 || b < 0 || a >= w->K || b >= w->K)
    return SAGE_E_INVALID;
  w->links.emplace_back(std::min(a, b), std::max(a, b));
  w->link_geo_loss.push_back(0.f);
  w->link_dense.push_back(dense);
  return (int)w->links.size() - 1;
}

extern "C" int sage_window_add_link(SageWindow *w, int a, int b) { return !w || w->finalized ? SAGE_E_INVALID : add_link(w, a, b, 1); }
extern "C" int sage_window_add_keypoint_link(SageWindow *w, int a, int b)
{
  return !w ? SAGE_E_INVALID : (w->finalized ? SAGE_E_STATE : add_link(w, a, b, 0));
}

extern "C" int sage_window_hold(SageWindow *w, int kf, int what)
{
  if (!w)
    return SAGE_E_INVALID;
  if (w->finalized)
    return SAGE_E_STATE;
  if (kf < 0 || kf >= w->K || what < 0 || what > (SAGE_HOLD_POSE | SAGE_HOLD_CODE | SAGE_HOLD_SCALE))
    return SAGE_E_INVALID;
  w->hold.resize(w->K, 0);
  w->hold[kf] = (uint8_t)what;
  return SAGE_OK;
}

extern "C" int sage_window_set_link_geo_loss(SageWindow *w, int link, float loss_param)
{
  if (!w || w->finalized || link < 0 || link >= (int)w->links.size() || !(loss_param >= 0.f))
    return w && w->finalized ? SAGE_E_STATE : SAGE_E_INVALID;
  w->link_geo_loss[link] = loss_param;
  return SAGE_OK;
}

static int photo_flush_for_runs(int tpb)
{
  if (const char *e = getenv("SAGE_PHOTO_FLUSH"))
    return std::max(0, atoi(e));
  return plan::record_cadence(tpb);
}

static int upload_work_list(DenseSide &sd, const WorkList &wl, hipStream_t s)
{
  int rc;
  sd.n_work = (int)wl.work.size();
  sd.tpb = wl.tiles_per_block;
  if ((rc = upload(sd.work, wl.work, s)) || (rc = upload(sd.first, wl.edge_first, s)) || (rc = upload(sd.tiles, wl.edge_tiles, s)))
    return rc;
  return SAGE_OK;
}

static void window_invalidate_plan_results(SageWindow *w)
{
  w->have_lin = false;
  w->spec_err_valid = false;
  w->dpt_set = -1;
}

static int window_plan_photo_runs(SageWindow *w, int tpb, int flush)
{
  WorkList wp;
  wp.build(w->Nedge, tpb, nullptr, flush);
  int rc;
  w->photo_rec.flush = wp.flush;
  w->photo_rec.n = wp.n_records;
  DenseSide &ph = w->dense[kPhoto];
  if ((rc = upload_work_list(ph, wp, w->stream)) || (rc = upload(w->photo_rec.first, wp.rec_first, w->stream)) ||
      (rc = upload(w->photo_rec.count, wp.rec_count, w->stream)))
    return rc;
  SAGE_HIP(hipStreamSynchronize(w->stream));
  return ph.part.reserve(std::max<size_t>(1, std::max(ph.n_work, w->photo_rec.n)) * photo_partial_floats(w->cfg.CS) * sizeof(float));
}

static std::vector<int> edge_tiles(const std::vector<int> &Nedge)
{
  std::vector<int> tiles;
  for (int n : Nedge)
    tiles.push_back((n + kTile - 1) / kTile);
  return tiles;
}

static int image_pixels(const SageWindow *w) { return (int)w->cfg.pyr.cam[0].h * (int)w->cfg.pyr.cam[0].w; }

static int finalize_variables(SageWindow *w)
{
  const int K = w->K, HW = image_pixels(w);
  int rc;
  for (int s = 0; s < 2; ++s)
  {
    if ((rc = w->vars[s].reserve((size_t)K * w->VS * sizeof(float))))
      return rc;
    if ((rc = window_upload_vars(w, s)))
      return rc;
  }
  if ((rc = w->dpt.reserve((size_t)K * HW * sizeof(float))) || (rc = w->dgrad.reserve((size_t)K * 2 * HW * sizeof(float))))
    return rc;
  return SAGE_OK;
}

static int finalize_ownership(SageWindow *w, FinalizeState &fs)
{
  const int K = w->K, HW = image_pixels(w);
  int rc;
  const bool by_link = sage::env_flag("SAGE_SHARD_BY_LINK") || fs.domain_solve;
  plan::Ownership own = plan::owned_edges((int)w->links.size(), w->rank, w->world, by_link);
  w->owned_edges = std::move(own.edges);
  w->local_links = std::move(own.links);
  w->local_edges = plan::dense_edges(w->owned_edges, w->link_dense);
  fs.needed.assign(K, 0);
  for (int ge : w->local_edges)
    fs.needed[w->links[ge / 2].first] = fs.needed[w->links[ge / 2].second] = 1;
  w->n_depth = 0;
  for (int k = 0; k < K; ++k)
    w->n_depth += fs.needed[k];
  for (int s = 0; s < 2; ++s)
  {
    std::vector<DepthItem> items;
    for (int k = 0; k < K; ++k)
    {
      if (!fs.needed[k])
        continue;
      const float *vp = w->vars[s].as<float>() + (size_t)k * w->VS;
      items.push_back(DepthItem{w->views[k].bias, w->views[k].basis, vp + 13, vp + 12,
                                w->dpt.as<float>() + (size_t)k * HW, w->dgrad.as<float>() + (size_t)k * 2 * HW});
    }
    if ((rc = upload(w->depth_items[s], items, w->stream)))
      return rc;
    SAGE_HIP(hipStreamSynchronize(w->stream));
  }
  return SAGE_OK;
}

static int finalize_pyramids(SageWindow *w)
{
  const SageWindowConfig &c = w->cfg;
  const int FS = c.FS, K = w->K;
  int rc;
  const size_t plane_f = (size_t)FS * c.pyr.P;
  if ((rc = w->pk.reserve((size_t)K * 3 * plane_f * sizeof(float))))
    return rc;
  float lvl_scale[SAGE_MAX_LEVELS] = {};
  for (int l = 0; l < c.pyr.levels; ++l)
  {
    if (!(c.photo_weights[l] >= 0.f))
      return SAGE_E_INVALID;
    lvl_scale[l] = std::sqrt(c.photo_weights[l]);
  }
  for (int k = 0; k < K; ++k)
  {
    float *base = w->pk.as<float>() + (size_t)k * 3 * plane_f;
    SAGE_HIP(launch_repack_groups(w->stream, base, w->views[k].feat_pyr, FS, c.pyr.P, 0, &c.pyr, lvl_scale));
    SAGE_HIP(launch_repack_groups(w->stream, base + plane_f, w->views[k].grad_pyr, FS, c.pyr.P, 1, &c.pyr, lvl_scale));
    SAGE_HIP(launch_repack_groups(w->stream, base + 2 * plane_f, w->views[k].grad_pyr + plane_f, FS, c.pyr.P, 2, &c.pyr, lvl_scale));
  }
// ... 202 lines not shown
  }
  return SAGE_OK;
}

static int finalize_work_lists(SageWindow *w, const FinalizeState &fs)
{
  const std::vector<int> tiles = edge_tiles(fs.Nedge);
  int rc;
  int tpb_g = plan::geo_run(plan::total_tiles(tiles));
  if (const char *e = getenv("SAGE_GEO_TPB"))
    tpb_g = std::max(1, atoi(e));
  WorkList wl;
  wl.build(fs.Nedge, tpb_g);
  if ((rc = upload_work_list(w->dense[kGeo], wl, w->stream)))
    return rc;
  SAGE_HIP(hipStreamSynchronize(w->stream));
  int tpb = plan::photo_run(tiles, w->cfg.FS);
  if (const char *e = getenv("SAGE_PHOTO_TPB"))
    tpb = std::max(1, atoi(e));
  w->Nedge = fs.Nedge;
  w->tpb_heur = tpb;
  if ((rc = window_plan_photo_runs(w, tpb, photo_flush_for_runs(tpb))))
    return rc;
  SAGE_HIP(hipStreamSynchronize(w->stream));
  return SAGE_OK;
}

static int finalize_results(SageWindow *w, const FinalizeState &fs)
{
  const int CS = w->cfg.CS, K = w->K;
  int rc;
  const size_t ne = std::max(1, w->n_edges);
  DenseSide &ph = w->dense[kPhoto], &ge = w->dense[kGeo];
  if ((rc = ph.reserve_results(ne, dense_dim(kPhoto, CS), std::max(ph.n_work, w->photo_rec.n), photo_partial_floats(CS))) ||
      (rc = ge.reserve_results(ne, dense_dim(kGeo, CS), ge.n_work, geo_partial_floats(CS))))
    return rc;
  std::vector<int32_t> adj_start(K + 1, 0);
  std::vector<AdjEntry> adj;
  for (int k = 0; k < K; ++k)
  {
    adj_start[k] = (int32_t)adj.size();
    adj.insert(adj.end(), fs.adjv[k].begin(), fs.adjv[k].end());
  }
  adj_start[K] = (int32_t)adj.size();
  if ((rc = upload(w->adj_start, adj_start, w->stream)) || (rc = upload(w->adj, adj, w->stream)) ||
      (rc = upload(w->link_edges, fs.le, w->stream)))
    return rc;
  SAGE_HIP(hipStreamSynchronize(w->stream));
  if ((rc = w->packed.reserve(sage_window_packed_count(w) * sizeof(double))) || (rc = w->errbuf.reserve(4 * sizeof(double))))
    return rc;
  {
    std::vector<int32_t> ids;
    for (int k = 0; k < K; ++k)
      if (!fs.adjv[k].empty())
        ids.push_back(k);
    for (size_t l = 0; l < fs.le.size(); ++l)
      if (fs.le[l].e_ab >= 0 || fs.le[l].e_ba >= 0 || fs.link_terms[l])
        ids.push_back(K + (int32_t)l);
    ids.push_back(K + (int32_t)w->links.size());
    w->dist.n_asm_blocks = (int)ids.size();
    if ((rc = upload(w->dist.asm_blocks, ids, w->stream)))
      return rc;
    SAGE_HIP(hipStreamSynchronize(w->stream));
  }
  SAGE_HIP(hipMemsetAsync(w->packed.p, 0, sage_window_packed_count(w) * sizeof(double), w->stream));
  SAGE_HIP(hipMemsetAsync(w->errbuf.p, 0, 4 * sizeof(double), w->stream));
  if (!w->mirror.h)
  {
    SAGE_HIP(hipHostMalloc(reinterpret_cast<void **>(&w->mirror.h), TotalsMirror::kDoubles * sizeof(double), hipHostMallocDefault));
    std::memset(w->mirror.h, 0, TotalsMirror::kDoubles * sizeof(double));
  }
  w->host_packed.assign(sage_window_packed_count(w), 0.0);
  w->delta.assign((size_t)K * w->B, 0.0);
  return SAGE_OK;
}

static int finalize_solver(SageWindow *w, const FinalizeState &fs)
{
  int rc = solver_create(&w->solver, w->K, w->rows, w->VS, w->links, w->stream);
  if (rc != SAGE_OK && rc != SAGE_E_UNSUPPORTED)
    return rc;
  if (w->solver && window_has_holds(w) && (rc = solver_set_holds(w->solver, w->hold, w->stream)))
    return rc;
  if (!fs.domain_solve)
    return SAGE_OK;
  const std::vector<int32_t> lk = window_link_pairs(w);
  if ((rc = sage_shard_plan_create(w->K, (int)w->links.size(), lk.data(), w->B, w->rank, w->world, &w->dist.shard)))
    return rc;
  const size_t ns = sage_shard_sep_count(w->dist.shard);
  w->dist.h_sep.assign(ns, 0.0);
  if ((rc = w->dist.sepbuf.reserve(ns * sizeof(double))))
    return rc;
  w->host_packed.resize(sage_window_packed_count(w));
  return SAGE_OK;
}

extern "C" int sage_window_finalize(SageWindow *w)
{
  if (!w || w->finalized || w->K < 1)
    return SAGE_E_INVALID;
  FinalizeState fs;
  const char *schur = getenv("SAGE_SHARD_SCHUR");
  fs.domain_solve = plan::uses_domain_solve(w->world, w->K, schur ? atoi(schur) != 0 : -1);
  w->hold.resize(w->K, 0);
  if (fs.domain_solve && (window_has_holds(w) || !w->terms.gt_added.empty()))
    return SAGE_E_UNSUPPORTED;
  w->rows = plan::solver_rows(w->hold.data(), w->K, w->cfg.CS);
  int rc;
  if ((rc = finalize_variables(w)) || (rc = finalize_ownership(w, fs)) || (rc = finalize_pyramids(w)) ||
      (rc = finalize_samples(w)) || (rc = finalize_source_features(w, fs)) || (rc = finalize_edge_tables(w, fs)) ||
      (rc = finalize_terms(w, fs)))
    return rc;
  w->residuals_per_lin = fs.residuals;
  w->bytes_per_lin = fs.bytes;
  if ((rc = finalize_work_lists(w, fs)) || (rc = finalize_results(w, fs)) || (rc = finalize_solver(w, fs)))
    return rc;
  w->finalized = true;
  if (const char *e = getenv("SAGE_AUTOTUNE"))
    if (atoi(e) != 0)
      return sage_window_tune_runs(w, nullptr, nullptr, nullptr, nullptr);
  return SAGE_OK;
}

extern "C" int sage_window_set_runs(SageWindow *w, int tpb)
{
  if (!w || !w->finalized)
    return SAGE_E_STATE;
  if (tpb < 1 || tpb > 64)
    return SAGE_E_INVALID;
  const int rc = window_plan_photo_runs(w, tpb, photo_flush_for_runs(tpb));
  window_invalidate_plan_results(w);
  return rc;
}

extern "C" int sage_window_tune_runs(SageWindow *w, int *tpb_out, int *tpb_rule_out, float *ms_rule_out, float *ms_best_out)
{
  if (!w || !w->finalized)
    return SAGE_E_STATE;
  const int rule = w->tpb_heur;
  if (tpb_out)
    *tpb_out = w->dense[kPhoto].tpb;
  if (tpb_rule_out)
    *tpb_rule_out = rule;
  if (ms_rule_out)
    *ms_rule_out = 0.f;
  if (ms_best_out)
    *ms_best_out = 0.f;
  if (getenv("SAGE_PHOTO_TPB") || w->world > 1 || w->dist.allreduce || w->n_edges == 0 || !(w->cfg.use_photo))
    return SAGE_OK;
  const std::vector<int> cand = plan::tune_candidates(rule, plan::typical_edge(edge_tiles(w->Nedge)));
  const bool prof_was = w->prof.profiling;
  const int level_was = w->prof.prof_level;
  int rc = sage_window_set_profiling(w, 1);
  double best_ms = 0.0, rule_ms = 0.0;
  int best = rule;
  auto measure = [&](int t, double &ms) -> int {
    int r = window_plan_photo_runs(w, t, photo_flush_for_runs(t));
    for (int rep = 0; rep < 4 && !r; ++rep)
    {
      if ((r = sage_window_linearize(w)) || (r = sage_window_error(w, 1)))
        break;
      double lin = 0.0, err = 0.0;
      int nl = 0, ne = 0;
      if ((r = sage_window_get_kernel_time(w, 0, &lin, &nl)) || (r = sage_window_get_kernel_time(w, 2, &err, &ne)))
        break;
      const double tt = lin / std::max(1, nl) + err / std::max(1, ne);
// ... 46 lines not shown
```

sage_slam_amd/csrc/window_eval.hip:

```cpp
#include "runtime_internal.h"
#include "finalize_bodies.h"

namespace sage
{

__device__ __forceinline__ int edge_col(int type, int role, int bi, int CS)
{
  if (bi < 6)
    return role * 6 + bi;
  if (type == 2)
    return bi == 6 + CS ? 12 + role : -1;
  if (type == 0)
  {
    if (role == 1)
      return -1;
    return bi < 6 + CS ? 12 + (bi - 6) : 12 + CS;
  }
  if (bi < 6 + CS)
    return 12 + role * CS + (bi - 6);
  return 12 + 2 * CS + role;
}

__device__ __forceinline__ double add_term_errors(double acc, const TermResults &r, bool photo, int lane)
{
// ... 64 lines not shown
#pragma unroll
    for (int s = 0; s < S; ++s)
    {
      const int idx = base + tfirst + s * tstride;
      if (!valid[s])
        continue;
      if (isg[s])
        g[(size_t)k * B + bi[s]] = acc[s];
      else
        diag[(size_t)k * BB + idx] = acc[s];
    }
    }
  }
  else if (blk < p.K + p.nlinks)
  {
    const int l = blk - p.K;
    const LinkEdges le = p.links[l];
    for (int idx = tfirst; idx < BB; idx += tstride)
    {
      const int bi = idx / B, bj = idx % B;
      double acc = 0.0;
      {
        for (int type = 0; type < 2; ++type)
        {
          if ((type == 0 && !p.AtA_p) || (type == 1 && !p.AtA_g))
            continue;
          const int D = type == 0 ? Dp : Dg;
          const float *A = type == 0 ? p.AtA_p : p.AtA_g;
          const double *Wd = type == 0 ? p.wide_p : p.wide_g;
          const size_t ws = (size_t)D * D + D;
          int ci = edge_col(type, 0, bi, p.CS), cj = edge_col(type, 1, bj, p.CS);
          if (le.e_ab >= 0 && ci >= 0 && cj >= 0)
            acc += Wd ? Wd[(size_t)le.e_ab * ws + (size_t)ci * D + cj] : (double)A[(size_t)le.e_ab * D * D + (size_t)ci * D + cj];
          ci = edge_col(type, 1, bi, p.CS);
          cj = edge_col(type, 0, bj, p.CS);
          if (le.e_ba >= 0 && ci >= 0 && cj >= 0)
            acc += Wd ? Wd[(size_t)le.e_ba * ws + (size_t)ci * D + cj] : (double)A[(size_t)le.e_ba * D * D + (size_t)ci * D + cj];
        }
      }
      if (KP && p.link_terms_start)
        for (int a = p.link_terms_start[l]; a < p.link_terms_start[l + 1]; ++a)
        {
          const AdjEntry ae = p.link_terms[a];
          const int lt = adj_group(ae.type), D = TermResults::dim(lt, p.CS);
          const float *A = p.terms.AtA(lt);
          const int ci = edge_col(lt, ae.role, bi, p.CS), cj = edge_col(lt, 1 - ae.role, bj, p.CS);
          if (ci >= 0 && cj >= 0)
            acc += (double)A[(size_t)ae.edge * D * D + (size_t)ci * D + cj];
        }
      lnk[(size_t)l * BB + idx] = acc;
    }
  }
  else
  {
    if (part != 0)
      return;
    const int wave = threadIdx.x >> 6, lane = threadIdx.x & 63;
    const bool photo = (wave & 1) == 0;
    const int which = wave >> 1;
    const float *st = photo ? p.stats_p : p.stats_g;
    const int n = photo ? p.n_edges_p : p.n_edges_g;
    double acc = 0.0;
    if (st && wave < 4)
      for (int e = lane; e < n; e += 64)
        acc += (double)st[2 * e + which];
    if (KP && p.terms.stats && wave < 2)
      acc = add_term_errors(acc, p.terms, photo, lane);
    for (int off = 32; off > 0; off >>= 1)
      acc += __shfl_down(acc, off);
    if (lane == 0 && wave < 4)
    {
      tail[which * 2 + (photo ? 0 : 1)] = acc;
      if (p.tail_mirror)
        p.tail_mirror[which * 2 + (photo ? 0 : 1)] = acc;
    }
  }
}

struct WindowFinalizeParams
{
  PhotoFinalizeParams ph;
  GeoFinalizeParams ge;
  int n_p, n_g;
};

template <int CS>
__global__ __launch_bounds__(kFinalizeBlock) void window_finalize_kernel(const WindowFinalizeParams prm)
{
  constexpr int LDS = photo_finalize_lds_doubles(CS) > geo_finalize_lds_doubles(CS) ? photo_finalize_lds_doubles(CS)
                                                                                    : geo_finalize_lds_doubles(CS);
  __shared__ double s[LDS];
  const int bid = (int)blockIdx.x;
  if (bid < prm.n_g)
    geo_finalize_body<CS>(prm.ge, bid, s);
  else
    photo_finalize_body<CS>(prm.ph, bid - prm.n_g, s);
}

template <bool KP>
__global__ __launch_bounds__(1024) void error_totals_kernel(const ErrorTotalsSide ph, const ErrorTotalsSide ge, double *out,
                                                            double *mirror, double epoch, const TermResults terms)
{
  for (int idx = threadIdx.x; idx < ph.n_edges + ge.n_edges; idx += blockDim.x)
  {
    const bool photo = idx < ph.n_edges;
    const ErrorTotalsSide &sd = photo ? ph : ge;
    const int e = photo ? idx : idx - ph.n_edges;
    const int first = sd.edge_first[e], nt = sd.edge_tiles[e];
    float se = 0.f, sn = 0.f;
    for (int t0 = 0; t0 < nt; t0 += 8)
    {
      float ve[8], vn[8];
#pragma unroll
      for (int u = 0; u < 8; ++u)
      {
        const int t = t0 + u < nt ? t0 + u : nt - 1;
        ve[u] = sd.partials[(size_t)(first + t) * sd.stride + sd.err_off];
        vn[u] = sd.partials[(size_t)(first + t) * sd.stride + sd.cnt_off];
      }
#pragma unroll
      for (int u = 0; u < 8; ++u)
        if (t0 + u < nt)
        {
          se += ve[u];
          sn += vn[u];
        }
    }
    sd.stats[2 * e + 0] = sn > 0.f ? sd.scale * se / sn : sd.fallback;
    sd.stats[2 * e + 1] = sn;
  }
  __threadfence_block();
  __syncthreads();
  const int wave = threadIdx.x >> 6, lane = threadIdx.x & 63;
  if (wave >= 4)
    return;
  const bool photo = (wave & 1) == 0;
  const int which = wave >> 1;
  const ErrorTotalsSide &sd = photo ? ph : ge;
  double acc = 0.0;
  for (int e0 = lane; e0 < sd.n_edges; e0 += 64 * 8)
  {
    float v[8];
#pragma unroll
    for (int u = 0; u < 8; ++u)
    {
      const int e = e0 + 64 * u;
      v[u] = sd.stats[2 * (e < sd.n_edges ? e : lane) + which];
    }
#pragma unroll
    for (int u = 0; u < 8; ++u)
      if (e0 + 64 * u < sd.n_edges)
        acc += (double)v[u];
  }
  if (KP && terms.stats && which == 0)
    acc = add_term_errors(acc, terms, photo, lane);
  for (int off = 32; off > 0; off >>= 1)
    acc += __shfl_down(acc, off);
  if (lane == 0)
  {
    out[which * 2 + (photo ? 0 : 1)] = acc;
    if (mirror)
    {
      mirror[which * 2 + (photo ? 0 : 1)] = acc;
      __threadfence_system();
      *reinterpret_cast<volatile double *>(mirror + 4 + which * 2 + (photo ? 0 : 1)) = epoch;
    }
  }
}

}

static LaunchCommon window_lc(SageWindow *w, int type, bool photo_linearize = false)
{
  const DenseSide &sd = w->dense[type];
  LaunchCommon lc{};
  lc.work = sd.work.as<WorkItem>();
  lc.edge_first = sd.first.as<int32_t>();
  lc.edge_tiles = sd.tiles.as<int32_t>();
  lc.n_work = sd.n_work;
  lc.n_edges = w->n_edges;
  lc.partials = sd.part.as<float>();
  lc.tiles_per_block = sd.tpb;
  lc.packed = type == kPhoto;
  if (photo_linearize && w->photo_rec.flush > 0)
  {
    lc.edge_first = w->photo_rec.first.as<int32_t>();
    lc.edge_tiles = w->photo_rec.count.as<int32_t>();
    lc.flush = w->photo_rec.flush;
  }
  return lc;
}

template <class E, class P>
static void finalize_side(P &fp, const DenseSide &sd, int set, const LaunchCommon &lc)
{
  const EdgeOut out = sd.out();
  fp.table = sd.tab[set].as<E>();
  fp.edge_first = lc.edge_first; fp.edge_tiles = lc.edge_tiles; fp.partials = lc.partials;
  fp.AtA = out.AtA; fp.Atb = out.Atb; fp.stats = out.stats; fp.wide = out.wide;
}

static float photo_weight_sum(const SageWindowConfig &c)
{
  float wsum = 0.f;
  for (int l = 0; l < c.pyr.levels; ++l)
    wsum += c.photo_weights[l];
  return wsum;
}

static AssembleParams window_assemble_params(SageWindow *w)
{
  const SageWindowConfig &c = w->cfg;
  AssembleParams ap{};
  const bool has = w->n_edges > 0;
  const EdgeOut op = w->dense[kPhoto].out(), og = w->dense[kGeo].out();
  ap.AtA_p = (has && c.use_photo) ? op.AtA : nullptr;
  ap.Atb_p = op.Atb;
  ap.stats_p = (has && c.use_photo) ? op.stats : nullptr;
  ap.wide_p = (has && c.use_photo) ? op.wide : nullptr;
  ap.AtA_g = (has && c.use_geo) ? og.AtA : nullptr;
  ap.Atb_g = og.Atb;
  ap.stats_g = (has && c.use_geo) ? og.stats : nullptr;
  ap.wide_g = (has && c.use_geo) ? og.wide : nullptr;
  ap.adj_start = w->adj_start.as<int32_t>();
  ap.adj = w->adj.as<AdjEntry>();
  ap.links = w->link_edges.as<LinkEdges>();
  ap.packed = w->packed.as<double>();
  ap.tail_mirror = w->kernels_mirror_totals() ? w->mirror.h + TotalsMirror::kTail : nullptr;
  ap.K = w->K;
  ap.nlinks = (int)w->links.size();
  ap.CS = c.CS;
  ap.n_edges_p = w->n_edges;
  ap.n_edges_g = w->n_edges;
  ap.split = 1;
  ap.blocks = nullptr;
  ap.terms = w->terms.results(true);
  ap.link_terms_start = w->terms.link_start.as<int32_t>();
  ap.link_terms = w->terms.link.as<AdjEntry>();
  return ap;
}

int window_linearize_set(SageWindow *w, int set, double *dst, bool local_blocks, bool merge)
{
  if (!w || !w->finalized)
    return SAGE_E_STATE;
  const SageWindowConfig &c = w->cfg;
  const int H = (int)c.pyr.cam[0].h, W = (int)c.pyr.cam[0].w;
  const bool dense = w->n_edges > 0;
  LaunchCommon lcg{}, lcp{};
  merge = merge && w->merge_ok;
  if (dense)
  {
    const bool have_depth = w->dpt_set == set;
    SAGE_HIP(launch_depth_batch(w->stream, c.CS, w->depth_items[set].as<DepthItem>(), w->n_depth, H, W, !have_depth,
                                !(have_depth && w->dgrad_valid)));
    w->dpt_set = set;
    w->dgrad_valid = true;
    lcg = window_lc(w, kGeo);
    lcp = window_lc(w, kPhoto, true);
    lcg.stage = 1;
    lcp.stage = 1;
    lcg.merge_geo_weight = lcp.merge_geo_weight = merge ? c.geo_weight : 0.f;
    if (c.use_geo)
    {
      prof_attach(w, 1, lcg);
      SAGE_HIP(launch_geo_linearize(w->stream, c.CS, nullptr, w->dense[kGeo].tab[set].as<GeoEdge>(), lcg, c.pyr.cam[0], c.eps,
                                    c.geo_loss_param, c.geo_weight, w->dense[kGeo].out()));
    }
    if (c.use_photo)
    {
      prof_attach(w, 0, lcp);
      SAGE_HIP(launch_photo_linearize(w->stream, c.CS, c.FS, nullptr, w->dense[kPhoto].tab[set].as<PhotoEdge>(), lcp, c.pyr,
                                      c.photo_weights, c.eps, w->dense[kPhoto].out()));
    }
  }
  if (const int rct = window_launch_terms(w, set, true))
    return rct;
  if (dense)
  {
    WindowFinalizeParams fp{};
    fp.n_p = c.use_photo ? w->n_edges : 0;
    fp.n_g = c.use_geo ? w->n_edges : 0;
    finalize_side<PhotoEdge>(fp.ph, w->dense[kPhoto], set, lcp);
    fp.ph.wsum = photo_weight_sum(c);
    finalize_side<GeoEdge>(fp.ge, w->dense[kGeo], set, lcg);
    fp.ge.weight = c.geo_weight;
    if (merge)
    {
      fp.ge.photo_partials = lcp.partials;
      fp.ge.photo_rec_first = lcp.edge_first;
      fp.ge.photo_rec_count = lcp.edge_tiles;
    }
    if (c.CS == 32)
      hipLaunchKernelGGL((window_finalize_kernel<32>), dim3(fp.n_p + fp.n_g), dim3(kFinalizeBlock), 0, w->stream, fp);
    else
      hipLaunchKernelGGL((window_finalize_kernel<16>), dim3(fp.n_p + fp.n_g), dim3(kFinalizeBlock), 0, w->stream, fp);
    SAGE_HIP(hipGetLastError());
  }
  AssembleParams ap = window_assemble_params(w);
  if (dst)
    ap.packed = dst;
  ap.split = 4;
  int nblocks = w->K + ap.nlinks + 1;
  if (local_blocks && w->dist.n_asm_blocks > 0)
  {
    ap.blocks = w->dist.asm_blocks.as<int32_t>();
    nblocks = w->dist.n_asm_blocks;
  }
  if (ap.terms.stats)
    hipLaunchKernelGGL(assemble_kernel<true>, dim3(nblocks * ap.split), dim3(512), 0, w->stream, ap);
  else
    hipLaunchKernelGGL(assemble_kernel<false>, dim3(nblocks * ap.split), dim3(512), 0, w->stream, ap);
  SAGE_HIP(hipGetLastError());
  window_phase_mark(w, 1);
  if (ap.packed == w->packed.as<double>())
  {
    w->have_lin = true;
    w->lin_epoch = set == 0 ? w->vars_epoch : 0;
    w->spec_err_valid = false;
    w->dist.packed_reduced = false;
  }
  return SAGE_OK;
}

extern "C" int sage_window_linearize(SageWindow *w)
{
  if (w)
    window_phase_mark(w, 0);
  return window_linearize_set(w, 0);
}

struct PartialRecord
{
  int stride, err_slot, cnt_slot;
};
constexpr PartialRecord kOwnRecord{2, 0, 1};
constexpr PartialRecord kFusedPhoto{4, 0, 1}, kFusedGeo{4, 2, 3};

static ErrorTotalsSide error_totals_side(const LaunchCommon &lc, float *stats, float fallback, float scale, int n_edges,
                                         PartialRecord rec)
{
  ErrorTotalsSide sd{};
  sd.edge_first = lc.edge_first; sd.edge_tiles = lc.edge_tiles; sd.partials = lc.partials;
  sd.stats = stats;
  sd.fallback = fallback; sd.scale = scale;
  sd.n_edges = n_edges;
  sd.stride = rec.stride; sd.err_off = rec.err_slot; sd.cnt_off = rec.cnt_slot;
  return sd;
}

int window_error_pass(SageWindow *w, int which, bool speculate_gradients)
{
  if (!w || !w->finalized || which < 0 || which > 1)
    return SAGE_E_STATE;
  const SageWindowConfig &c = w->cfg;
  const int H = (int)c.pyr.cam[0].h, W = (int)c.pyr.cam[0].w;
  const bool has = w->n_edges > 0;
  if (has && w->dpt_set != which)
  {
    SAGE_HIP(launch_depth_batch(w->stream, c.CS, w->depth_items[which].as<DepthItem>(), w->n_depth, H, W, true, false));
    w->dpt_set = which;
    w->dgrad_valid = false;
  }
  ErrorTotalsSide ph{}, ge{};
  const bool fused = has && c.use_photo && c.use_geo;
  if (has && c.use_photo)
  {
    LaunchCommon lc = window_lc(w, kPhoto);
    prof_attach(w, 2, lc);
    lc.stage = 1;
    lc.fused_geo_loss_param = fused ? c.geo_loss_param : 0.f;
    SAGE_HIP(launch_photo_error(w->stream, c.CS, c.FS, nullptr, w->dense[kPhoto].tab[which].as<PhotoEdge>(), lc, c.pyr,
                                c.photo_weights, c.eps, w->dense[kPhoto].stats.as<float>()));
    ph = error_totals_side(lc, w->dense[kPhoto].stats.as<float>(), 10.0f * photo_weight_sum(c), 1.0f, w->n_edges,
                           fused ? kFusedPhoto : kOwnRecord);
    if (fused)
      ge = error_totals_side(lc, w->dense[kGeo].stats.as<float>(), 10.0f * c.geo_weight, c.geo_weight, w->n_edges, kFusedGeo);
  }
  if (has && c.use_geo && !fused)
  {
    LaunchCommon lc = window_lc(w, kGeo);
    prof_attach(w, 3, lc);
    lc.stage = 1;
    SAGE_HIP(launch_geo_error(w->stream, c.CS, nullptr, w->dense[kGeo].tab[which].as<GeoEdge>(), lc, c.pyr.cam[0], c.eps,
                              c.geo_loss_param, c.geo_weight, w->dense[kGeo].stats.as<float>()));
    ge = error_totals_side(lc, w->dense[kGeo].stats.as<float>(), 10.0f * c.geo_weight, c.geo_weight, w->n_edges, kOwnRecord);
  }
  if (const int rct = window_launch_terms(w, which, false))
    return rct;
  const TermResults kpt = w->terms.results(false);
  w->mirror.err_epoch += 1;
  double *const mirror = w->kernels_mirror_totals() ? w->mirror.h + TotalsMirror::kError : nullptr;
  if (kpt.stats)
    hipLaunchKernelGGL(error_totals_kernel<true>, dim3(1), dim3(1024), 0, w->stream, ph, ge, w->errbuf.as<double>(), mirror,
                       (double)w->mirror.err_epoch, kpt);
  else
    hipLaunchKernelGGL(error_totals_kernel<false>, dim3(1), dim3(1024), 0, w->stream, ph, ge, w->errbuf.as<double>(), mirror,
                       (double)w->mirror.err_epoch, kpt);
  SAGE_HIP(hipGetLastError());
  window_phase_mark(w, 4);
  if (speculate_gradients && has && c.use_geo && w->dpt_set == which && !w->dgrad_valid)
  {
    SAGE_HIP(launch_depth_batch(w->stream, c.CS, w->depth_items[which].as<DepthItem>(), w->n_depth, H, W, false, true));
// ... 7 lines not shown
```

sage_slam_amd/csrc/window_lm.hip:

```cpp
#include "runtime_internal.h"

enum class LmSeq { classic, schur, at_candidate };

static LmSeq lm_sequence_for(const SageWindow *w, const SageLmConfig *cfg)
{
  const bool sharded = w->dist.allreduce != nullptr;
  if (sharded && w->dist.shard)
    return LmSeq::schur;
  const bool at_candidate = cfg->linearize_at_candidate > 0 || (cfg->linearize_at_candidate == 0 && sharded);
  return at_candidate && !w->links.empty() ? LmSeq::at_candidate : LmSeq::classic;
}

struct LmEval
{
  double cur_tot[4];
  bool have_cur_tot;
};

static int window_form_system(SageWindow *w, int set, double *dst, int it)
{
  int rc;
  if (!w->dist.allreduce)
    return (rc = window_linearize_set(w, set, dst, false, true)) ? rc : window_mirror_totals(w, false, dst);
  if ((rc = window_linearize_set(w, set, w->dist.packed_loc.as<double>(), true, true)) ||
// ... 30 lines not shown
    if ((rc = window_form_system(w, 0, w->packed.as<double>(), w->dist.emu_cur)))
      return rc;
    w->have_lin = true;
    w->lin_epoch = w->vars_epoch;
    w->dist.packed_reduced = true;
    w->spec_err_valid = false;
    mirrored_now = true;
  }
  if (!w->spec_err_valid)
  {
    if (!mirrored_now && (rc = window_mirror_totals(w, false)))
      return rc;
    if (!window_wait_reduced_totals(w))
      SAGE_HIP(hipStreamSynchronize(w->stream));
    w->spec_error = mirrored_error(w, TotalsMirror::kTail, 0);
    w->spec_err_valid = true;
  }
  st->error = w->spec_error;
  return SAGE_OK;
}

static int evaluate_schur(SageWindow *w, SageLmState *st, bool first)
{
  int rc;
  double lin_error = 0;
  if ((rc = window_schur_solve(w, st->damp, &lin_error)) && rc != SAGE_E_NOT_PSD)
    return rc;
  window_phase_mark(w, 3);
  if (first)
    st->error = lin_error;
  st->candidate_error = INFINITY;
  if (rc == SAGE_E_NOT_PSD)
    return SAGE_OK;
  if ((rc = sage_window_error(w, 1)))
    return rc;
  window_add_to_double(w, w->errbuf.as<double>(), window_prior_error(w, 1, true));
  if ((rc = window_collective(w, w->errbuf.as<double>(), 4)))
    return rc;
  double t4[4];
  SAGE_HIP(hipMemcpyAsync(t4, w->errbuf.p, sizeof(t4), hipMemcpyDeviceToHost, w->stream));
  SAGE_HIP(hipStreamSynchronize(w->stream));
  st->candidate_error = t4[0] + t4[1];
  return SAGE_OK;
}

static int evaluate_at_candidate(SageWindow *w, SageLmState *st, LmEval &ev)
{
  int rc;
  std::memcpy(ev.cur_tot, w->mirror.h, sizeof(ev.cur_tot));
  ev.have_cur_tot = true;
  bool not_psd;
  if ((rc = window_form_system(w, 1, w->packed_save.as<double>(), w->dist.emu_cur + 1)) ||
      (rc = window_wait_mirror(w, &not_psd)))
    return rc;
  st->candidate_error = not_psd ? INFINITY : mirrored_error(w, TotalsMirror::kTail, 1);
  return SAGE_OK;
}

static int evaluate_classic(SageWindow *w, SageLmState *st, bool first)
{
  int rc;
  const bool sharded = w->dist.allreduce != nullptr;
  if ((rc = window_error_pass(w, 1, !sharded)))
    return rc;
  if (!sharded)
  {
    const bool idle = window_wait_error_totals(w);
    if (first && (rc = window_total_error(w, 1, &st->error, idle)))
      return rc;
    if ((rc = window_total_error(w, 0, &st->candidate_error, idle)) == SAGE_E_NOT_PSD)
      st->candidate_error = INFINITY;
    return rc == SAGE_E_NOT_PSD ? SAGE_OK : rc;
  }
  bool not_psd;
  if ((rc = window_allreduce(w, w->errbuf.as<double>(), 4, w->dist.emu_cur + 1)) || (rc = window_mirror_totals(w, true)) ||
      (rc = window_wait_mirror(w, &not_psd)))
    return rc;
  if (first)
    st->error = mirrored_error(w, TotalsMirror::kTail, 0);
  st->candidate_error = not_psd ? INFINITY : mirrored_error(w, TotalsMirror::kError, 1);
  return SAGE_OK;
}

static int lm_evaluate(LmSeq seq, SageWindow *w, SageLmState *st, bool first, LmEval &ev)
{
  if (seq == LmSeq::schur)
    return evaluate_schur(w, st, first);
  const int rc = sage_window_solve(w, st->damp, nullptr);
  if (rc == SAGE_E_NOT_PSD)
  {
    st->candidate_error = INFINITY;
    return first && seq == LmSeq::classic ? sage_window_total_error(w, 1, &st->error) : SAGE_OK;
  }
  if (rc)
    return rc;
  return seq == LmSeq::at_candidate ? evaluate_at_candidate(w, st, ev) : evaluate_classic(w, st, first);
}

static int lm_accept(LmSeq seq, SageWindow *w, const SageLmState *st)
{
  const int rc = sage_window_accept(w);
  if (rc || seq != LmSeq::at_candidate)
    return rc;
  w->packed.swap(w->packed_save);
  w->lin_epoch = w->vars_epoch;
  w->dist.packed_reduced = true;
  w->spec_error = st->candidate_error;
  return SAGE_OK;
}

static void lm_reject(SageWindow *w, const LmEval &ev)
{
  if (ev.have_cur_tot)
    std::memcpy(w->mirror.h, ev.cur_tot, sizeof(ev.cur_tot));
}

extern "C" int sage_window_lm_step(SageWindow *w, SageLmState *st, const SageLmConfig *cfg)
{
  if (!w || !st || !cfg)
    return SAGE_E_INVALID;
  if (w->world > 1 && !w->dist.allreduce)
    return SAGE_E_STATE;
  const LmSeq seq = lm_sequence_for(w, cfg);
  auto clampd = [&](double d) { return std::min(std::max((double)cfg->min_damp, d), (double)cfg->max_damp); };
  if (st->iters == 0 && st->damp <= 0)
    st->damp = cfg->init_damp;
  window_phase_mark(w, 0);
  int rc = lm_prepare(seq, w, st);
  if (rc)
    return rc;
  st->accepted = 0;
  for (int evals = 1;; ++evals)
  {
    LmEval ev{};
    if ((rc = lm_evaluate(seq, w, st, evals == 1, ev)))
      return rc;
    if (st->candidate_error < st->error)
    {
      st->accepted = 1;
      if ((rc = lm_accept(seq, w, st)))
        return rc;
      st->damp = clampd(st->damp / cfg->damp_dec_factor);
      break;
    }
    lm_reject(w, ev);
    const bool give_up = st->damp >= cfg->max_damp || (cfg->max_inner_evals > 0 && evals >= cfg->max_inner_evals);
    st->damp = clampd(st->damp * cfg->damp_inc_factor);
    if (give_up)
      break;
  }
  st->iters += 1;
  return SAGE_OK;
}

static int window_lm_run(SageWindow *w, SageLmState *st, const SageLmConfig *cfg, int n, double *trace, int *done,
                         double *step_seconds)
{
  if (!w || !st || !cfg || n < 0)
    return SAGE_E_INVALID;
  int i = 0, rc = SAGE_OK;
  auto t_prev = std::chrono::steady_clock::now();
  for (; i < n; ++i)
  {
    if ((rc = sage_window_lm_step(w, st, cfg)))
      break;
    if (trace)
    {
      trace[4 * i + 0] = st->error;
      trace[4 * i + 1] = st->candidate_error;
      trace[4 * i + 2] = (double)st->accepted;
      trace[4 * i + 3] = st->damp;
    }
    if (step_seconds)
    {
      const auto t = std::chrono::steady_clock::now();
      step_seconds[i] = std::chrono::duration<double>(t - t_prev).count();
      t_prev = t;
    }
  }
  if (done)
    *done = i;
  return rc;
}

extern "C" int sage_window_lm_run(SageWindow *w, SageLmState *st, const SageLmConfig *cfg, int n, double *trace, int *done)
{
  return window_lm_run(w, st, cfg, n, trace, done, nullptr);
}

extern "C" int sage_window_lm_run_timed(SageWindow *w, SageLmState *st, const SageLmConfig *cfg, int n, double *trace,
                                        int *done, double *step_seconds)
{
  return window_lm_run(w, st, cfg, n, trace, done, step_seconds);
}
```

sage_slam_amd/csrc/window_profile.hip:

```cpp
#include "runtime_internal.h"

WindowProfiler::~WindowProfiler()
{
  for (auto &pm : phase_pending)
    for (auto &m : pm.ev)
      (void)hipEventDestroy(m.second);
  for (auto &m : phase_cur.ev)
    (void)hipEventDestroy(m.second);
  for (auto &pend : pending)
    for (auto &pr : pend)
    {
      (void)hipEventDestroy(pr.first);
      (void)hipEventDestroy(pr.second);
    }
  for (hipEvent_t e : ev_free)
    (void)hipEventDestroy(e);
}

static bool ev_get(WindowProfiler &pf, hipEvent_t *e)
{
  if (!pf.ev_free.empty())
  {
    *e = pf.ev_free.back();
    pf.ev_free.pop_back();
    return true;
  }
  return hipEventCreate(e) == hipSuccess;
}
static void ev_put(WindowProfiler &pf, hipEvent_t e)
{
  if (e)
    pf.ev_free.push_back(e);
}

void prof_attach(SageWindow *w, int which, LaunchCommon &lc)
{
  WindowProfiler &pf = w->prof;
  if (!pf.profiling || (pf.prof_level == 2 && which != 0))
    return;
  hipEvent_t a, b;
  if (!ev_get(pf, &a))
    return;
  if (!ev_get(pf, &b))
  {
    ev_put(pf, a);
    return;
  }
  lc.ev_start = a;
  lc.ev_stop = b;
  pf.pending[which].emplace_back(a, b);
}

void window_phase_mark(SageWindow *w, int which)
{
  WindowProfiler &pf = w->prof;
  if (!pf.profiling || pf.prof_level == 2)
    return;
  if (which == 0)
  {
    if (pf.phase_cur.ev.size() >= 2)
    {
      if (pf.phase_pending.size() >= 1024)
      {
        for (auto &m : pf.phase_pending.front().ev)
          ev_put(pf, m.second);
        pf.phase_pending.erase(pf.phase_pending.begin());
      }
      pf.phase_pending.push_back(std::move(pf.phase_cur));
    }
    else
      for (auto &m : pf.phase_cur.ev)
        ev_put(pf, m.second);
    pf.phase_cur = WindowProfiler::PhaseMarks{};
  }
  else if (pf.phase_cur.ev.empty())
    return;
  hipEvent_t e;
  if (pf.phase_cur.ev.size() >= 64 || !ev_get(pf, &e))
    return;
  (void)hipEventRecord(e, w->stream);
  pf.phase_cur.ev.emplace_back(which, e);
}

extern "C" int sage_window_get_phase_time(SageWindow *w, double *ms4, int *iterations)
{
  if (!w || !ms4)
    return SAGE_E_INVALID;
  WindowProfiler &pf = w->prof;
  SAGE_HIP(hipStreamSynchronize(w->stream));
  window_phase_mark(w, 0);
  for (auto &m : pf.phase_cur.ev)
    ev_put(pf, m.second);
  pf.phase_cur = WindowProfiler::PhaseMarks{};
  for (auto &pm : pf.phase_pending)
  {
    double d4[4] = {0, 0, 0, 0};
    bool ok = true;
    for (size_t i = 1; i < pm.ev.size() && ok; ++i)
    {
      float d = 0.f;
      ok = hipEventElapsedTime(&d, pm.ev[i - 1].second, pm.ev[i].second) == hipSuccess;
      const int ph = pm.ev[i].first;
      if (ok && ph >= 1 && ph <= 4)
        d4[ph - 1] += d;
    }
    if (ok)
    {
      for (int i = 0; i < 4; ++i)
        pf.phase_ms[i] += d4[i];
      pf.phase_n += 1;
    }
    for (auto &m : pm.ev)
      ev_put(pf, m.second);
  }
  pf.phase_pending.clear();
  for (int i = 0; i < 4; ++i)
  {
    ms4[i] = pf.phase_ms[i];
    pf.phase_ms[i] = 0;
  }
  if (iterations)
    *iterations = pf.phase_n;
  pf.phase_n = 0;
  return SAGE_OK;
}

extern "C" int sage_window_set_profiling(SageWindow *w, int on)
{
  if (!w)
    return SAGE_E_INVALID;
  WindowProfiler &pf = w->prof;
  pf.profiling = on != 0;
  pf.prof_level = on;
  while (pf.profiling && pf.ev_free.size() < 512)
  {
    hipEvent_t e;
    if (hipEventCreate(&e) != hipSuccess)
      break;
    pf.ev_free.push_back(e);
  }
  return SAGE_OK;
}

extern "C" int sage_window_get_kernel_time(SageWindow *w, int which, double *total_ms, int *launches)
{
  if (!w || which < 0 || which > 7)
    return SAGE_E_INVALID;
  WindowProfiler &pf = w->prof;
  SAGE_HIP(hipStreamSynchronize(w->stream));
  for (auto &pr : pf.pending[which])
  {
    float ms = 0.f;
    if (hipEventElapsedTime(&ms, pr.first, pr.second) == hipSuccess)
    {
      pf.prof_ms[which] += ms;
      pf.prof_n[which] += 1;
    }
    ev_put(pf, pr.first);
    ev_put(pf, pr.second);
  }
  pf.pending[which].clear();
  if (total_ms)
    *total_ms = pf.prof_ms[which];
  if (launches)
    *launches = pf.prof_n[which];
  pf.prof_ms[which] = 0;
  pf.prof_n[which] = 0;
  return SAGE_OK;
}
```

sage_slam_amd/csrc/window_solve.hip:

```cpp
#include "damped_system.h"
#include "runtime_internal.h"

double window_prior_error(const SageWindow *w, int set, bool owned_only)
{
  const SageWindowConfig &c = w->cfg;
  double e = 0;
  auto keyframe0_terms = [&] {
    if (c.scale_prior_weight > 0)
    {
      const double d = std::log((double)w->hv.scale_init[0]) - std::log((double)w->hv.scale[set][0]);
      e += c.scale_prior_weight * d * d;
    }
    if (c.pose_prior_weight > 0)
    {
      double loc[6];
      sage::pose_local(&w->hv.pose[set][0], &w->hv.pose_init[0], loc);
      for (int i = 0; i < 6; ++i)
        e += c.pose_prior_weight * loc[i] * loc[i];
    }
  };
  for (int k = 0; k < w->K; ++k)
  {
    if (owned_only && sage_shard_keyframe_owner(w->dist.shard, k) != w->rank)
      continue;
// ... 76 lines not shown
extern "C" int sage_window_solve(SageWindow *w, double damp, double *step_norm)
{
  if (!w || !w->finalized || !w->have_lin)
    return SAGE_E_STATE;
  const SageWindowConfig &c = w->cfg;
  const int K = w->K, B = w->B, CS = c.CS;
  if (w->solver)
  {
    int rc = window_sync_candidate(w);
    if (rc && rc != SAGE_E_NOT_PSD)
      return rc;
    if (w->dpt_set == 1)
      w->dpt_set = -1;
    rc = solver_run(w->solver, w->stream, w->packed.as<double>(), w->vars[0].as<float>(), w->vars[1].as<float>(), CS,
                    damp, window_solve_priors(w));
    if (rc)
      return rc;
    window_phase_mark(w, 3);
    w->cand_pending = true;
    if (step_norm)
    {
      if ((rc = window_sync_candidate(w)))
        return rc;
      *step_norm = std::sqrt(solver_host_step_norm2(w->solver));
    }
    return SAGE_OK;
  }
  const size_t np = sage_window_packed_count(w);
  static const bool dbg = sage::env_flag("SAGE_DEBUG_TIMING");
  auto tnow = [] { return std::chrono::steady_clock::now(); };
  auto t_a = tnow();
  SAGE_HIP(hipStreamSynchronize(w->stream));
  auto t_b = tnow();
  SAGE_HIP(hipMemcpyAsync(w->host_packed.data(), w->packed.p, np * sizeof(double), hipMemcpyDeviceToHost, w->stream));
  SAGE_HIP(hipStreamSynchronize(w->stream));
  auto t_c = tnow();
  std::vector<double> dadd, gadd;
  window_priors(w, dadd, gadd);
  const std::vector<int32_t> lk = window_link_pairs(w);
  const bool holds = window_has_holds(w);
  if (holds)
    sage::hold_packed(w->host_packed.data(), dadd.data(), gadd.data(), K, (int)w->links.size(), lk.data(), B, CS, w->hold.data());
  int rcs;
  if (w->rows.compact())
  {
    const int Bs = w->rows.Bs, nl = (int)w->links.size();
    std::vector<double> ps((size_t)(K + nl) * Bs * Bs + (size_t)K * Bs);
    std::vector<double> ds((size_t)K * Bs), gs((size_t)K * Bs), xs((size_t)K * Bs);
    sage::compact_packed(w->host_packed.data(), dadd.data(), gadd.data(), K, nl, B, Bs, w->rows.to_block.data(), ps.data(),
                         ds.data(), gs.data());
    if ((rcs = sage_block_solve(ps.data(), K, nl, lk.data(), Bs, damp, ds.data(), gs.data(), xs.data())))
      return rcs;
    std::fill(w->delta.begin(), w->delta.end(), 0.0);
    for (int k = 0; k < K; ++k)
      for (int s = 0; s < Bs; ++s)
        w->delta[(size_t)k * B + w->rows.to_block[s]] = xs[(size_t)k * Bs + s];
  }
  else if ((rcs = sage_block_solve(w->host_packed.data(), K, (int)w->links.size(), lk.data(), B, damp, dadd.data(),
                                   gadd.data(), w->delta.data())))
    return rcs;
  if (holds)
    for (int k = 0; k < K; ++k)
      for (int r = 0; r < B; ++r)
        if (sage::row_held(w->hold[k], r, CS))
          w->delta[(size_t)k * B + r] = 0.0;
  auto t_d = tnow();
  double nrm = 0;
  for (double v : w->delta)
    nrm += v * v;
  if (step_norm)
    *step_norm = std::sqrt(nrm);
  window_retract_candidate(w, false);
  const int rcu = window_upload_vars(w, 1);
  if (dbg)
  {
    auto t_e = tnow();
    auto ms = [](auto a, auto b) { return std::chrono::duration<double, std::milli>(b - a).count(); };
    fprintf(stderr, "[sage solve] wait-kernels %.3f d2h %.3f block_solve %.3f retract+h2d %.3f ms\n", ms(t_a, t_b),
            ms(t_b, t_c), ms(t_c, t_d), ms(t_d, t_e));
  }
  return rcu;
}

int window_schur_solve(SageWindow *w, double damp, double *lin_error)
{
  const int K = w->K, B = w->B;
  const size_t np = sage_window_packed_count(w), ns = w->dist.h_sep.size();
  SAGE_HIP(hipMemcpyAsync(w->host_packed.data(), w->packed.p, np * sizeof(double), hipMemcpyDeviceToHost, w->stream));
  SAGE_HIP(hipStreamSynchronize(w->stream));
  std::vector<double> dadd, gadd;
  window_priors(w, dadd, gadd);
  int rc = sage_shard_eliminate(w->dist.shard, w->host_packed.data(), damp, dadd.data(), gadd.data(), w->dist.h_sep.data());
  if (rc && rc != SAGE_E_NOT_PSD)
    return rc;
  if (rc == SAGE_E_NOT_PSD)
  {
    std::fill(w->dist.h_sep.begin(), w->dist.h_sep.end() - 8, 0.0);
    w->dist.h_sep[ns - 3] = 1.0;
  }
  w->dist.h_sep[ns - 4] = window_prior_error(w, 0, true);
  SAGE_HIP(hipMemcpyAsync(w->dist.sepbuf.p, w->dist.h_sep.data(), ns * sizeof(double), hipMemcpyHostToDevice, w->stream));
  if ((rc = window_collective(w, w->dist.sepbuf.as<double>(), ns)))
    return rc;
  SAGE_HIP(hipMemcpyAsync(w->dist.h_sep.data(), w->dist.sepbuf.p, ns * sizeof(double), hipMemcpyDeviceToHost, w->stream));
  SAGE_HIP(hipStreamSynchronize(w->stream));
  if (lin_error)
    *lin_error = w->dist.h_sep[ns - 8] + w->dist.h_sep[ns - 7] + w->dist.h_sep[ns - 4];
  if (w->dist.h_sep[ns - 3] > 0.0 || std::isnan(w->dist.h_sep[0]))
    return SAGE_E_NOT_PSD;
  w->delta.assign((size_t)K * B, 0.0);
  rc = sage_shard_solve(w->dist.shard, w->dist.h_sep.data(), w->delta.data());
  if (rc)
    return rc;
  window_retract_candidate(w, true);
  w->cand_pending = false;
  return window_upload_vars(w, 1);
}

extern "C" int sage_window_accept(SageWindow *w)
{
  if (!w || !w->finalized)
    return SAGE_E_STATE;
  int rcs = window_sync_candidate(w);
  if (rcs)
    return rcs;
  w->hv.copy_set(0, 1);
  ++w->vars_epoch;
  ++w->dist.emu_cur;
  w->dpt_set = w->dpt_set == 1 ? 0 : -1;
  return window_copy_floats(w, w->vars[1].as<float>(), w->vars[0].as<float>(), w->K * w->VS);
}

extern "C" int sage_window_reset(SageWindow *w)
{
  if (!w || !w->finalized)
    return SAGE_E_STATE;
  (void)window_sync_candidate(w);
  for (int s = 0; s < 2; ++s)
  {
    w->hv.pose[s] = w->hv.pose_init;
    w->hv.code[s] = w->hv.code_added;
    w->hv.scale[s] = w->hv.scale_init;
  }
  int rc;
  if ((rc = window_upload_vars(w, 0)) || (rc = window_upload_vars(w, 1)))
    return rc;
  w->have_lin = false;
  w->dist.emu_cur = 0;
  return SAGE_OK;
}

extern "C" int sage_window_sync_variables(SageWindow *w)
{
  if (!w || !w->finalized)
    return SAGE_E_STATE;
  if (!w->dist.shard)
    return SAGE_OK;
  if (!w->dist.allreduce)
    return SAGE_E_STATE;
  const int K = w->K, CS = w->cfg.CS, VS = 13 + CS;
  std::vector<double> buf((size_t)K * VS, 0.0);
  for (int k = 0; k < K; ++k)
    if (sage_shard_keyframe_owner(w->dist.shard, k) == w->rank)
      w->hv.pack(0, k, CS, &buf[(size_t)k * VS]);
  int rc;
  {
// ... 28 lines not shown
```

sage_slam_amd/csrc/window_state.h:

```cpp
#pragma once

namespace sage_rt
{

enum : int { kPhoto = 0, kGeo = 1 };

static inline size_t dense_dim(int type, int CS) { return type == kPhoto ? 13 + (size_t)CS : 14 + 2 * (size_t)CS; }

struct HostVars
{
  std::vector<float> pose[2], code[2], scale[2];
  std::vector<float> code_init, scale_init, pose_init;
  std::vector<float> code_added;
  void copy_set(int dst, int src) { pose[dst] = pose[src], code[dst] = code[src], scale[dst] = scale[src]; }

  template <class T>
  void pack(int set, int k, int CS, T *rec) const
  {
    for (int i = 0; i < 12; ++i)
      rec[i] = pose[set][(size_t)k * 12 + i];
    rec[12] = scale[set][k];
    for (int i = 0; i < CS; ++i)
      rec[13 + i] = code[set][(size_t)k * CS + i];
  }
// ... 2 lines not shown
  {
    for (int i = 0; i < 12; ++i)
      pose[set][(size_t)k * 12 + i] = (float)rec[i];
    scale[set][k] = (float)rec[12];
    for (int i = 0; i < CS; ++i)
      code[set][(size_t)k * CS + i] = (float)rec[13 + i];
  }
};

struct DenseSide
{
  DevBuf tab[2];
  DevBuf work, first, tiles;
  DevBuf part;
  DevBuf AtA, Atb, stats;
  DevBuf wide;
  int n_work = 0, tpb = 1;
  EdgeOut out() const { return EdgeOut{AtA.as<float>(), Atb.as<float>(), stats.as<float>(), wide.as<double>()}; }
  int reserve_results(size_t ne, size_t D, size_t records, size_t partial_floats)
  {
    int rc;
    if ((rc = part.reserve(std::max<size_t>(1, records) * partial_floats * sizeof(float))) ||
        (rc = AtA.reserve(ne * D * D * sizeof(float))) || (rc = Atb.reserve(ne * D * sizeof(float))) ||
        (rc = stats.reserve(ne * 2 * sizeof(float))) || (rc = wide.reserve(ne * (D * D + D) * sizeof(double))))
      return rc;
    return 0;
  }
};

struct KeypointTermHost
{
  int32_t kind, edge, N, loss;
  float loss_param, weight;
  std::vector<int32_t> loc0, loc1;
  std::vector<float> homo0, second;
  std::vector<float> dpts0, dpts1;
};
struct TermSide
{
  std::vector<KeypointTermHost> kp_added;
  std::vector<SageGraphTerm> gt_added;
  plan::TermLayout layout;
  DevBuf pool, kp_table, gt_table;
  DevBuf link_start, link;
  DevBuf AtA[plan::kTermGroups], Atb[plan::kTermGroups];
  DevBuf stats;
  bool linearized = false;
  int n_keypoint() const { return layout.n_keypoint(); }
  int n_graph() const { return layout.n_graph(); }
  int n_stats() const { return layout.n_stats(); }
  unsigned keypoint_kinds() const
  {
    unsigned m = 0;
    for (int id : layout.kp_order)
      m |= 1u << kp_added[id].kind;
    return m;
  }
  TermResults results(bool jac) const
  {
    float *st = n_stats() ? stats.as<float>() + (jac ? 0 : (size_t)2 * n_stats()) : nullptr;
    return TermResults{AtA[0].as<float>(), Atb[0].as<float>(), AtA[1].as<float>(), Atb[1].as<float>(), AtA[2].as<float>(),
                       Atb[2].as<float>(), st, layout.count[0], layout.count[1], layout.count[2]};
  }
  int reserve_results(int CS, hipStream_t s)
  {
    const size_t bytes = (size_t)2 * n_stats() * 2 * sizeof(float);
    int rc = stats.reserve(bytes);
    for (int g = 0; g < plan::kTermGroups && !rc; ++g)
    {
      const size_t n = std::max(1, layout.count[g]), D = TermResults::dim(g, CS);
      if (!(rc = AtA[g].reserve(n * D * D * sizeof(float))))
        rc = Atb[g].reserve(n * D * sizeof(float));
    }
    return rc ? rc : (int)hipMemsetAsync(stats.p, 0, bytes, s);
  }
};

struct PhotoRecordPlan
{
  DevBuf first, count;
  int flush = 0, n = 0;
};

struct TotalsMirror
{
  enum : int { kTail = 0, kError = 4, kErrorTickets = 8, kMirrorTickets = 12, kDoubles = 16 };
  double *h = nullptr;
  uint64_t err_epoch = 0;
  uint64_t mirror_epoch = 0;
  TotalsMirror() = default;
  TotalsMirror(const TotalsMirror &) = delete;
  TotalsMirror &operator=(const TotalsMirror &) = delete;
  ~TotalsMirror()
  {
    if (h)
      (void)hipHostFree(h);
  }
  bool wait(int ticket_group, uint64_t epoch) const
  {
    const double *t = h + ticket_group;
    const double want = (double)epoch;
    auto ticket = [t](int i) {
      double v;
      __atomic_load(t + i, &v, __ATOMIC_ACQUIRE);
      return v;
    };
    const auto t0 = std::chrono::steady_clock::now();
    unsigned spins = 0;
    while (!(ticket(0) == want && ticket(1) == want && ticket(2) == want && ticket(3) == want))
    {
      __builtin_ia32_pause();
      if ((++spins & 0x3ff) == 0 &&
          std::chrono::duration<double>(std::chrono::steady_clock::now() - t0).count() > 0.05)
        return false;
    }
    std::atomic_thread_fence(std::memory_order_acquire);
    return true;
  }
};

struct WindowDist
{
  SageAllReduceFn allreduce = nullptr;
  int (*allreduce2)(const double *send, double *recv, size_t n, void *user) = nullptr;
  void *allreduce_user = nullptr;
  void *rccl_hook = nullptr;
  SageShardPlan *shard = nullptr;
  DevBuf sepbuf;
  std::vector<double> h_sep;
  const double *emu_rest = nullptr;
  int emu_n = 0, emu_cur = 0;
  DevBuf packed_loc;
  DevBuf asm_blocks;
  int n_asm_blocks = 0;
  bool packed_reduced = false;
};

struct WindowProfiler
{
  struct PhaseMarks
  {
    std::vector<std::pair<int, hipEvent_t>> ev;
  };
  std::vector<PhaseMarks> phase_pending;
  PhaseMarks phase_cur;
  double phase_ms[4] = {0, 0, 0, 0};
  int phase_n = 0;
  bool profiling = false;
  int prof_level = 0;
  std::vector<std::pair<hipEvent_t, hipEvent_t>> pending[8];
  std::vector<hipEvent_t> ev_free;
  double prof_ms[8] = {0, 0, 0, 0, 0, 0, 0, 0};
  int prof_n[8] = {0, 0, 0, 0, 0, 0, 0, 0};
  WindowProfiler() = default;
  WindowProfiler(const WindowProfiler &) = delete;
  WindowProfiler &operator=(const WindowProfiler &) = delete;
  ~WindowProfiler();
};

}
```

Before: 260,800 Mresiduals/s.

## Split linearization into two parts overlapped with block solve consumption order

Plans a split of photometric work items, edges and assembly blocks into a part A (touching the first tA rows of each half of the block elimination order) and a part B. The first LM evaluation then runs a combined linearize+solve, where the solver starts factorizing the rows fed by part A while part B is linearized and assembled. The aim is to hide linearization latency behind the block factorization instead of running them one after another. It adds planning code, extra launches for finalize and assemble, and only applies on the single-GPU, photo-only path without keypoint or graph terms.

New measurement: 256,300 Mresiduals/s. -1.7%, worse.

```diff
diff --git a/include/sage_ba.h b/include/sage_ba.h
--- a/include/sage_ba.h
+++ b/include/sage_ba.h
@@ -116,6 +116,10 @@
 int sage_block_solve(const double *packed_host, int K, int nlinks, const int32_t *links, int B, double damp,
                      const double *diag_add, const double *g_add, double *delta);
 long long sage_solve_lookahead_count(void);
+int sage_plan_split(int K, int nlinks, const int32_t *links, int n_items, const int32_t *item_edge, int slots, int force_tA,
+                    int32_t *tA, int32_t *scatterA, int32_t *order, int32_t *edgesA, int32_t *edgesB, int32_t *blocksA,
+                    int32_t *blocksB, int32_t *workA, int32_t *workB, int32_t *perm, int32_t *blk_row, int32_t *blk_col,
+                    int32_t *blk_src);
 
 typedef struct SageLmConfig
 {
@@ -387,6 +391,7 @@
 int sage_window_lm_run(SageWindow *w, SageLmState *st, const SageLmConfig *cfg, int n, double *trace, int *done);
 int sage_window_lm_run_timed(SageWindow *w, SageLmState *st, const SageLmConfig *cfg, int n, double *trace, int *done,
                              double *step_seconds);
+int sage_window_split_rows(const SageWindow *w);
 int sage_window_sync_variables(SageWindow *w);
 
 #ifdef __cplusplus
diff --git a/sage_slam_amd/build.py b/sage_slam_amd/build.py
--- a/sage_slam_amd/build.py
+++ b/sage_slam_amd/build.py
@@ -12,7 +12,7 @@
 LIB = os.path.join(HERE, "libsage_ba.so")
 SOURCES = ["photo_kernels.hip", "geo_kernels.hip", "track_kernels.hip", "producers.hip", "keypoint_kernels.hip", "graph_kernels.hip", "solve_kernels.hip", "operators.hip", "tracker.hip", "overlap.hip", "window.hip", "window_eval.hip", "window_reduce.hip", "window_solve.hip", "window_lm.hip", "window_profile.hip", "window_build.hip", "window_terms.hip", "window_dist.hip", "window_factors.hip",
            "host_math.cpp", "block_solver.cpp", "host_threads.cpp", "shard_solve.cpp", "convex_hull.cpp"]
-HEADERS = ["sage_device.h", "sage_internal.h", "damped_system.h", "host_math.h", "block_solver.h", "host_threads.h", "runtime_internal.h", "window_state.h", "finalize_bodies.h", "keypoint_batch.h", "graph_terms.h", "graph_batch.h", "term_results.h", "window_plan.h", os.path.join(ROOT, "include", "sage_ba.h")]
+HEADERS = ["sage_device.h", "sage_internal.h", "damped_system.h", "host_math.h", "block_solver.h", "solve_parts.h", "host_threads.h", "runtime_internal.h", "window_state.h", "finalize_bodies.h", "keypoint_batch.h", "graph_terms.h", "graph_batch.h", "term_results.h", "window_plan.h", os.path.join(ROOT, "include", "sage_ba.h")]
 HIPCC = os.environ.get("HIPCC", "/opt/rocm/bin/hipcc")
 HOSTCXX = os.environ.get("HOSTCXX", "/opt/rocm/lib/llvm/bin/clang++")
 FLAGS = ["--offload-arch=gfx950", "-O3", "-std=c++17", "-fPIC", "-Wall", "-Wno-unused-function",
diff --git a/sage_slam_amd/capi.py b/sage_slam_amd/capi.py
--- a/sage_slam_amd/capi.py
+++ b/sage_slam_amd/capi.py
@@ -124,14 +124,14 @@
     "sage_tracker_photo_jac_error_calculate", "sage_tracker_photo_error_calculate",
     "sage_geometric_jac_error_calculate", "sage_geometric_error_calculate", "sage_depth_and_grad",
     "sage_gaussian_pyramid_with_grad", "sage_se3_exp", "sage_pose_retract", "sage_nearest_psd", "sage_nearest_psd_reference", "sage_factor_block_count", "sage_factor_hessian_blocks",
-    "sage_damped_solve_qr_f32", "sage_block_solve", "sage_solve_lookahead_count", "sage_lm_config_default", "sage_track_lm", "sage_track_frame", "sage_track_overlap", "sage_convex_hull_area",
+    "sage_damped_solve_qr_f32", "sage_block_solve", "sage_solve_lookahead_count", "sage_plan_split", "sage_lm_config_default", "sage_track_lm", "sage_track_frame", "sage_track_overlap", "sage_convex_hull_area",
     "sage_window_create", "sage_window_destroy", "sage_window_add_keyframe", "sage_window_add_link", "sage_window_add_keypoint_link", "sage_window_hold", "sage_window_set_link_geo_loss",
     "sage_window_set_shard", "sage_window_finalize", "sage_window_num_keyframes", "sage_window_num_links",
     "sage_window_block_size", "sage_window_solver_block_size", "sage_window_packed_count", "sage_window_packed_dev",
     "sage_window_residuals_per_linearize", "sage_window_bytes_per_linearize", "sage_window_linearize",
     "sage_window_error", "sage_window_tune_runs", "sage_window_set_runs", "sage_window_error_dev", "sage_window_solve", "sage_window_total_error",
     "sage_window_accept", "sage_window_reset", "sage_window_get_keyframe", "sage_window_set_keyframe", "sage_window_get_delta",
-    "sage_window_get_edge", "sage_window_add_keypoint_term", "sage_window_num_keypoint_terms", "sage_window_get_keypoint_term", "sage_window_add_graph_term", "sage_window_num_graph_terms", "sage_window_get_graph_term", "sage_window_prepass", "sage_window_factor", "sage_window_factor_error", "sage_window_prepare_factors", "sage_factor_psd", "sage_factor_cut_blocks", "sage_window_set_profiling", "sage_window_get_kernel_time", "sage_window_get_phase_time", "sage_window_lm_step", "sage_window_lm_run", "sage_window_lm_run_timed", "sage_window_sync_variables", "sage_window_set_allreduce", "sage_shard_plan_create", "sage_shard_plan_create_domains", "sage_block_solve_domains", "sage_shard_plan_destroy", "sage_shard_sep_count", "sage_shard_num_separators", "sage_shard_num_interior", "sage_shard_keyframe_owner", "sage_shard_keyframe_is_local", "sage_shard_eliminate", "sage_shard_solve", "sage_rccl_unique_id", "sage_rccl_comm_create", "sage_rccl_comm_destroy", "sage_rccl_comm_info", "sage_window_use_rccl", "sage_window_emulate_peers", "sage_sort_locations", "sage_bind_thread_to_device", "sage_solver_helper_cpus", "sage_solver_placement_moves", "sage_placement_monitor", "sage_shutdown", "sage_host_threads_running",
+    "sage_window_get_edge", "sage_window_add_keypoint_term", "sage_window_num_keypoint_terms", "sage_window_get_keypoint_term", "sage_window_add_graph_term", "sage_window_num_graph_terms", "sage_window_get_graph_term", "sage_window_prepass", "sage_window_factor", "sage_window_factor_error", "sage_window_prepare_factors", "sage_factor_psd", "sage_factor_cut_blocks", "sage_window_set_profiling", "sage_window_get_kernel_time", "sage_window_get_phase_time", "sage_window_lm_step", "sage_window_lm_run", "sage_window_lm_run_timed", "sage_window_split_rows", "sage_window_sync_variables", "sage_window_set_allreduce", "sage_shard_plan_create", "sage_shard_plan_create_domains", "sage_block_solve_domains", "sage_shard_plan_destroy", "sage_shard_sep_count", "sage_shard_num_separators", "sage_shard_num_interior", "sage_shard_keyframe_owner", "sage_shard_keyframe_is_local", "sage_shard_eliminate", "sage_shard_solve", "sage_rccl_unique_id", "sage_rccl_comm_create", "sage_rccl_comm_destroy", "sage_rccl_comm_info", "sage_window_use_rccl", "sage_window_emulate_peers", "sage_sort_locations", "sage_bind_thread_to_device", "sage_solver_helper_cpus", "sage_solver_placement_moves", "sage_placement_monitor", "sage_shutdown", "sage_host_threads_running",
     "sage_valid_locations", "sage_shuffle_indices", "sage_sample_locations",
     "sage_reprojection_jac_error_calculate", "sage_reprojection_error_calculate",
     "sage_tracker_reproj_jac_error_calculate", "sage_tracker_reproj_error_calculate",
@@ -262,6 +262,22 @@
                                 C.c_double(damp), dp(da), dp(ga), delta.ctypes.data_as(C.POINTER(C.c_double))),
          "sage_block_solve")
     return delta
+
+
+def plan_split(K, links, item_edge, slots, force_tA=0):
+    lk = np.ascontiguousarray(np.asarray(links, dtype=np.int32).reshape(-1))
+    ie = np.ascontiguousarray(np.asarray(item_edge, dtype=np.int32).reshape(-1))
+    nl = len(lk) // 2
+    ip = lambda a: a.ctypes.data_as(C.POINTER(C.c_int32))
+    tA, sc = C.c_int32(0), C.c_int32(0)
+    cap = K * K + K + 2 * nl + len(ie) + 2
+    names = ("order", "edgesA", "edgesB", "blocksA", "blocksB", "workA", "workB", "perm", "blk_row", "blk_col", "blk_src")
+    bufs = {n: np.zeros(cap, np.int32) for n in names}
+    _chk(lib().sage_plan_split(K, nl, ip(lk), len(ie), ip(ie), int(slots), int(force_tA), C.byref(tA), C.byref(sc),
+                               *[ip(bufs[n]) for n in names]), "sage_plan_split")
+    out = {n: bufs[n][1:1 + bufs[n][0]].copy() for n in names}
+    out["tA"], out["scatterA"] = int(tA.value), int(sc.value)
+    return out
 
 
 def solve_lookahead_count() -> int:
@@ -748,6 +764,9 @@
         _chk(lib().sage_window_lm_step(self.h, C.byref(state), C.byref(cfg)), "sage_window_lm_step")
         return state
 
+    def split_rows(self) -> int:
+        return int(lib().sage_window_split_rows(self.h))
+
     def lm_run(self, state: SageLmState, cfg: SageLmConfig, n: int):
         tr = np.zeros((n, 4), np.float64)
         done = C.c_int()
diff --git a/sage_slam_amd/csrc/block_solver.cpp b/sage_slam_amd/csrc/block_solver.cpp
--- a/sage_slam_amd/csrc/block_solver.cpp
+++ b/sage_slam_amd/csrc/block_solver.cpp
@@ -1604,6 +1604,150 @@
   env.col_ptr = plan.col_ptr.data(); env.col_rows = plan.col_rows.data();
   return env;
 }
+
+static std::vector<int32_t> consumption_prefix(const BlockPlan &plan, int rows_per_half)
+{
+  const int K = (int)plan.row_first.size(), n1 = plan.n1, n2 = plan.n2;
+  std::vector<int32_t> order;
+  auto push_row = [&](int i) {
+    for (int q = 0; q < plan.a_cnt[i]; ++q)
+      order.push_back(plan.a_off[i] + q);
+    for (int q = 0; q <= i - plan.row_first[i]; ++q)
+      order.push_back(plan.row_off[i] + q);
+  };
+  if (n1 > 0)
+  {
+    const int tmax = std::max(n1, n2);
+    for (int t = 0; t < (rows_per_half > 0 ? std::min(rows_per_half, tmax) : tmax); ++t)
+    {
+      if (t < n1)
+        push_row(t);
+      if (t < n2)
+        push_row(n1 + t);
+    }
+    if (rows_per_half <= 0)
+      for (int i = n1 + n2; i < K; ++i)
+        push_row(i);
+  }
+  else if (rows_per_half <= 0)
+    for (int i = 0; i < K; ++i)
+      push_row(i);
+  return order;
+}
+
+std::vector<int32_t> consumption_order(const BlockPlan &plan) { return consumption_prefix(plan, 0); }
+
+bool plan_split(const BlockPlan &plan, const std::vector<std::pair<int, int>> &links, const std::vector<int32_t> &item_edge,
+                int slots, int force_tA, SplitPlan &out)
+{
+  out = SplitPlan();
+  const int K = (int)plan.row_first.size(), nl = (int)links.size(), n1 = plan.n1, n2 = plan.n2;
+  if (n1 < 1 || n2 < 1 || slots < 1 || block_plan_has_arrow_rows(envelope_of(plan, 0)))
+    return false;
+  std::vector<long long> items(2 * (size_t)nl, 0);
+  for (int32_t e : item_edge)
+  {
+    if (e < 0 || e >= 2 * nl)
+      return false;
+    ++items[e];
+  }
+  const long long total = (long long)item_edge.size();
+  auto in_rows = [&](int k, int t) {
+    const int p = plan.pos[k];
+    return p < n1 ? p < t : (p < n1 + n2 && p - n1 < t);
+  };
+  auto is_A = [&](int l, int t) { return in_rows(links[l].first, t) || in_rows(links[l].second, t); };
+  auto rounds = [&](long long n) { return (n + slots - 1) / slots; };
+  int best = 0;
+  long long best_cost = 0;
+  for (int t = 1; t <= std::max(n1, n2); ++t)
+  {
+    long long nA = 0;
+    int linksA = 0;
+    for (int l = 0; l < nl; ++l)
+      if (is_A(l, t))
+      {
+        nA += items[2 * l] + items[2 * l + 1];
+        ++linksA;
+      }
+    if (linksA == nl)
+      break;
+    if (linksA == 0)
+      continue;
+    if (force_tA > 0)
+    {
+      if (t <= force_tA)
+        best = t;
+      continue;
+    }
+    const long long nB = total - nA;
+    if (4 * nB < 3 * (long long)slots)
+      continue;
+    const long long cost = rounds(nA) + rounds(nB);
+    if (best == 0 || cost <= best_cost)
+    {
+      best = t;
+      best_cost = cost;
+    }
+  }
+  if (best == 0)
+    return false;
+  out.tA = best;
+  out.scatterA = (int)consumption_prefix(plan, best).size();
+  std::vector<char> edge_in_A(2 * (size_t)nl, 0), all_A(K, 1);
+  for (int l = 0; l < nl; ++l)
+  {
+    const bool a = is_A(l, best);
+    edge_in_A[2 * l] = edge_in_A[2 * l + 1] = a;
+    for (int d = 0; d < 2; ++d)
+      (a ? out.edgesA : out.edgesB).push_back(2 * l + d);
+    if (!a)
+      all_A[links[l].first] = all_A[links[l].second] = 0;
+  }
+  for (int k = 0; k < K; ++k)
+    (all_A[k] ? out.blocksA : out.blocksB).push_back(k);
+  for (int l = 0; l < nl; ++l)
+    (edge_in_A[2 * l] ? out.blocksA : out.blocksB).push_back(K + l);
+  out.blocksB.push_back(K + nl);
+  for (size_t i = 0; i < item_edge.size(); ++i)
+    (edge_in_A[item_edge[i]] ? out.workA : out.workB).push_back((int32_t)i);
+  return true;
+}
+}
+
+extern "C" int sage_plan_split(int K, int nlinks, const int32_t *links, int n_items, const int32_t *item_edge, int slots,
+                               int force_tA, int32_t *tA, int32_t *scatterA, int32_t *order, int32_t *edgesA, int32_t *edgesB,
+                               int32_t *blocksA, int32_t *blocksB, int32_t *workA, int32_t *workB, int32_t *perm,
+                               int32_t *blk_row, int32_t *blk_col, int32_t *blk_src)
+{
+  if (K < 1 || nlinks < 0 || n_items < 0 || (nlinks > 0 && !links) || (n_items > 0 && !item_edge))
+    return SAGE_E_INVALID;
+  std::vector<std::pair<int, int>> lk(nlinks);
+  for (int l = 0; l < nlinks; ++l)
+    lk[l] = {links[2 * l], links[2 * l + 1]};
+  sage::BlockPlan bp;
+  const int rcp = sage::plan_blocks(K, lk, !sage::env_flag("SAGE_SOLVE_NO_SPLIT"), bp);
+  if (rcp != SAGE_OK)
+    return rcp;
+  sage::SplitPlan sp;
+  sage::plan_split(bp, lk, std::vector<int32_t>(item_edge, item_edge + n_items), slots, force_tA, sp);
+  auto put = [](int32_t *dst, const std::vector<int32_t> &v) {
+    if (!dst)
+      return;
+    dst[0] = (int32_t)v.size();
+    std::copy(v.begin(), v.end(), dst + 1);
+  };
+  if (tA)
+    *tA = sp.tA;
+  if (scatterA)
+    *scatterA = sp.scatterA;
+  put(order, sage::consumption_order(bp));
+  put(edgesA, sp.edgesA); put(edgesB, sp.edgesB);
+  put(blocksA, sp.blocksA); put(blocksB, sp.blocksB);
+  put(workA, sp.workA); put(workB, sp.workB);
+  put(perm, bp.perm);
+  put(blk_row, bp.blk_row); put(blk_col, bp.blk_col); put(blk_src, bp.blk_src);
+  return SAGE_OK;
 }
 
 extern "C" long long sage_solve_lookahead_count(void) { return sage::g_lookahead_count.load(); }
diff --git a/sage_slam_amd/csrc/block_solver.h b/sage_slam_amd/csrc/block_solver.h
--- a/sage_slam_amd/csrc/block_solver.h
+++ b/sage_slam_amd/csrc/block_solver.h
@@ -80,4 +80,16 @@
 };
 int plan_blocks(int K, const std::vector<std::pair<int, int>> &links, bool may_split, BlockPlan &out);
 BlockEnvelope envelope_of(const BlockPlan &plan, int Bp);
+std::vector<int32_t> consumption_order(const BlockPlan &plan);
+
+struct SplitPlan
+{
+  int tA = 0;
+  int scatterA = 0;
+  std::vector<int32_t> edgesA, edgesB;
+  std::vector<int32_t> blocksA, blocksB;
+  std::vector<int32_t> workA, workB;
+};
+bool plan_split(const BlockPlan &plan, const std::vector<std::pair<int, int>> &links, const std::vector<int32_t> &item_edge,
+                int slots, int force_tA, SplitPlan &out);
 }
diff --git a/sage_slam_amd/csrc/runtime_internal.h b/sage_slam_amd/csrc/runtime_internal.h
--- a/sage_slam_amd/csrc/runtime_internal.h
+++ b/sage_slam_amd/csrc/runtime_internal.h
@@ -35,6 +35,7 @@
 #include "host_threads.h"
 #include "sage_ba.h"
 #include "sage_internal.h"
+#include "solve_parts.h"
 #include "keypoint_batch.h"
 #include "graph_batch.h"
 #include "window_plan.h"
@@ -249,6 +250,7 @@
   DevBuf f0s;
   DenseSide dense[2];
   PhotoRecordPlan photo_rec;
+  LinearizeSplit split;
   std::vector<int> Nedge;
   int tpb_heur = 1;
   DevBuf adj_start, adj, link_edges, packed, errbuf;
@@ -313,6 +315,8 @@
 int window_launch_terms(SageWindow *w, int set, bool jac);
 int window_linearize_set(SageWindow *w, int set, double *dst = nullptr, bool local_blocks = false, bool merge = false);
 int window_error_pass(SageWindow *w, int which, bool speculate_gradients);
+bool window_split_applies(const SageWindow *w);
+int window_linearize_part(SageWindow *w, int part);
 int window_collective(SageWindow *w, double *buf, size_t n);
 int window_allreduce(SageWindow *w, double *buf, size_t n, int iterate);
 int window_allreduce_into(SageWindow *w, const double *send, double *recv, size_t n, int iterate);
@@ -327,5 +331,7 @@
 double window_prior_error(const SageWindow *w, int set, bool owned_only = false);
 int window_sync_candidate(SageWindow *w, bool stream_idle = false);
 int window_schur_solve(SageWindow *w, double damp, double *lin_error);
-void prof_attach(SageWindow *w, int which, LaunchCommon &lc);
+int window_linearize_solve(SageWindow *w, double damp);
+int window_plan_split(SageWindow *w);
+void prof_attach(SageWindow *w, int which, LaunchCommon &lc, bool joined = false);
 void window_phase_mark(SageWindow *w, int which);
diff --git a/sage_slam_amd/csrc/solve_kernels.hip b/sage_slam_amd/csrc/solve_kernels.hip
--- a/sage_slam_amd/csrc/solve_kernels.hip
+++ b/sage_slam_amd/csrc/solve_kernels.hip
@@ -11,6 +11,7 @@
 #include "host_math.h"
 #include "sage_device.h"
 #include "sage_internal.h"
+#include "solve_parts.h"
 #include "window_plan.h"
 
 namespace sage
@@ -42,8 +43,8 @@
                                                             const float *__restrict__ vars0, int VS, int CS,
                                                             const SolvePriors pri, double damp,
                                                             double *__restrict__ L, double *__restrict__ y,
-                                                            const int32_t *__restrict__ order, unsigned *flags,
-                                                            unsigned epoch)
+                                                            const int32_t *__restrict__ order, int first, int count,
+                                                            unsigned *flags, unsigned epoch)
 {
   const int tid = threadIdx.x;
   const int B = P.B, Bs = P.Bs, Bp = P.Bp, BB = B * B;
@@ -52,7 +53,7 @@
   if (tid < Bs)
     s_row[tid] = P.to_block[tid];
   __syncthreads();
-  for (int it = blockIdx.x; it < P.nblk; it += gridDim.x)
+  for (int it = first + blockIdx.x; it < first + count; it += gridDim.x)
   {
     const int b = order[it];
     const int i = P.blk_row[b], j = P.blk_col[b], srcf = P.blk_src[b];
@@ -245,10 +246,9 @@
   const int rcp = plan_blocks(K, links, !sage::env_flag("SAGE_SOLVE_NO_SPLIT"), bp);
   if (rcp != SAGE_OK)
     return rcp;
-  const int n1 = bp.n1, n2 = bp.n2, nblk = bp.nblk;
+  const int nblk = bp.nblk;
   const std::vector<int32_t> &perm = bp.perm, &pos = bp.pos, &row_first = bp.row_first, &row_off = bp.row_off,
-                             &a_cnt = bp.a_cnt, &a_off = bp.a_off, &blk_row = bp.blk_row, &blk_col = bp.blk_col,
-                             &blk_src = bp.blk_src;
+                             &blk_row = bp.blk_row, &blk_col = bp.blk_col, &blk_src = bp.blk_src;
   std::unique_ptr<DeviceSolver> S(new DeviceSolver);
   S->K = K; S->B = B; S->Bs = Bs; S->Bp = Bp; S->nblk = nblk; S->nlinks = (int)links.size(); S->VS = VS;
   std::vector<int32_t> all;
@@ -261,28 +261,7 @@
   };
   const size_t o_rf = put(row_first), o_ro = put(row_off), o_br = put(blk_row), o_bc = put(blk_col),
                o_bs = put(blk_src), o_pm = put(perm), o_ps = put(pos);
-  std::vector<int32_t> order;
-  auto push_row = [&](int i) {
-    for (int q = 0; q < a_cnt[i]; ++q)
-      order.push_back(a_off[i] + q);
-    for (int q = 0; q <= i - row_first[i]; ++q)
-      order.push_back(row_off[i] + q);
-  };
-  if (n1 > 0)
-  {
-    for (int t = 0; t < std::max(n1, n2); ++t)
-    {
-      if (t < n1)
-        push_row(t);
-      if (t < n2)
-        push_row(n1 + t);
-    }
-    for (int i = n1 + n2; i < K; ++i)
-      push_row(i);
-  }
-  else
-    for (int i = 0; i < K; ++i)
-      push_row(i);
+  const std::vector<int32_t> order = consumption_order(bp);
   const size_t o_ord = put(order);
   const size_t o_tb = put(rows.to_block), o_ts = put(rows.to_solver);
   if (hipMalloc(&S->d_int, all.size() * sizeof(int32_t)) != hipSuccess)
@@ -337,6 +316,20 @@
 int solver_run(DeviceSolver *S, hipStream_t stream, const double *packed_dev, const float *vars0, float *vars1,
                int CS, double damp, const SolvePriors &pri)
 {
+  return solver_run_parts(S, stream, packed_dev, vars0, vars1, CS, damp, pri, 0, nullptr, nullptr);
+}
+
+bool solver_plan_split(const DeviceSolver *S, const std::vector<std::pair<int, int>> &links,
+                       const std::vector<int32_t> &item_edge, int slots, int force_tA, SplitPlan &out)
+{
+  return plan_split(S->host_plan, links, item_edge, slots, force_tA, out);
+}
+
+int solver_run_parts(DeviceSolver *S, hipStream_t stream, const double *packed_dev, const float *vars0, float *vars1, int CS,
+                     double damp, const SolvePriors &pri, int scatterA, SolverProduceFn produce, void *user)
+{
+  if (produce && (scatterA < 1 || scatterA >= S->nblk))
+    return SAGE_E_INVALID;
   static const bool dbgt = sage::env_flag("SAGE_DEBUG_TIMING");
   hipError_t eh;
   SolveLease lease;
@@ -346,11 +339,29 @@
   S->epoch += 1;
   if (S->epoch == 0)
     S->epoch = 1;
-  hipLaunchKernelGGL(solve_scatter_kernel, dim3(std::min(kScatterWorkgroups, S->nblk)), dim3(256), 0, stream, S->plan,
-                     packed_dev, vars0, S->VS, CS, pri, damp, reinterpret_cast<double *>(S->h_T), S->h_y, S->d_order,
-                     S->h_flags, S->epoch);
-  if ((eh = hipGetLastError()) != hipSuccess)
-    return (int)eh;
+  auto scatter = [&](int first, int count) {
+    hipLaunchKernelGGL(solve_scatter_kernel, dim3(std::min(kScatterWorkgroups, count)), dim3(256), 0, stream, S->plan,
+                       packed_dev, vars0, S->VS, CS, pri, damp, reinterpret_cast<double *>(S->h_T), S->h_y, S->d_order, first,
+                       count, S->h_flags, S->epoch);
+    return hipGetLastError();
+  };
+  int rcp;
+  if (!produce)
+  {
+    if ((eh = scatter(0, S->nblk)) != hipSuccess)
+      return (int)eh;
+  }
+  else
+  {
+    if ((rcp = produce(user, 0)))
+      return rcp;
+    if ((eh = scatter(0, scatterA)) != hipSuccess)
+      return (int)eh;
+    if ((rcp = produce(user, 1)))
+      return rcp;
+    if ((eh = scatter(scatterA, S->nblk - scatterA)) != hipSuccess)
+      return (int)eh;
+  }
   volatile unsigned *go = &S->result()->go;
   S->go_epoch = (S->go_epoch + 1) & 0x7fffffffu;
   if (S->go_epoch == 0)
diff --git a/sage_slam_amd/csrc/solve_parts.h b/sage_slam_amd/csrc/solve_parts.h
--- /dev/null
+++ b/sage_slam_amd/csrc/solve_parts.h
@@ -0,0 +1,17 @@
+#pragma once
+#include <hip/hip_runtime.h>
+
+#include <utility>
+#include <vector>
+
+#include "block_solver.h"
+#include "sage_internal.h"
+
+namespace sage
+{
+bool solver_plan_split(const DeviceSolver *S, const std::vector<std::pair<int, int>> &links,
+                       const std::vector<int32_t> &item_edge, int slots, int force_tA, SplitPlan &out);
+typedef int (*SolverProduceFn)(void *user, int part);
+int solver_run_parts(DeviceSolver *S, hipStream_t stream, const double *packed_dev, const float *vars0, float *vars1, int CS,
+                     double damp, const SolvePriors &pri, int scatterA, SolverProduceFn produce, void *user);
+}
diff --git a/sage_slam_amd/csrc/window_build.hip b/sage_slam_amd/csrc/window_build.hip
--- a/sage_slam_amd/csrc/window_build.hip
+++ b/sage_slam_amd/csrc/window_build.hip
@@ -122,6 +122,49 @@
   w->dpt_set = -1;
 }
 
+int window_plan_split(SageWindow *w)
+{
+  LinearizeSplit &sp = w->split;
+  sp.tA = sp.scatterA = 0;
+  const char *env = getenv("SAGE_LIN_SPLIT");
+  const int force = !env ? 0 : (std::strcmp(env, "auto") == 0 ? -1 : atoi(env));
+  if (force == 0 || !w->solver || w->world != 1 || w->n_edges == 0 || w->n_edges != 2 * (int)w->links.size() ||
+      !w->terms.kp_added.empty() || !w->terms.gt_added.empty())
+    return SAGE_OK;
+  int dev = 0, cus = 0;
+  if (hipGetDevice(&dev) != hipSuccess || hipDeviceGetAttribute(&cus, hipDeviceAttributeMultiprocessorCount, dev) != hipSuccess || cus < 1)
+    return SAGE_OK;
+  WorkList wp;
+  wp.build(w->Nedge, w->dense[kPhoto].tpb);
+  std::vector<int32_t> item_edge;
+  for (const WorkItem &wi : wp.work)
+    item_edge.push_back(wi.edge);
+  SplitPlan plan;
+  if (!solver_plan_split(w->solver, w->links, item_edge, 3 * cus, std::max(force, 0), plan))
+    return SAGE_OK;
+  int rc;
+  for (int part = 0; part < 2; ++part)
+  {
+    std::vector<WorkItem> items;
+    for (int32_t i : part == 0 ? plan.workA : plan.workB)
+      items.push_back(wp.work[i]);
+    const std::vector<int32_t> &edges = part == 0 ? plan.edgesA : plan.edgesB;
+    const std::vector<int32_t> &blocks = part == 0 ? plan.blocksA : plan.blocksB;
+    if (items.empty() || edges.empty() || blocks.empty())
+      return SAGE_OK;
+    sp.n_work[part] = (int)items.size();
+    sp.n_edges[part] = (int)edges.size();
+    sp.n_blocks[part] = (int)blocks.size();
+    if ((rc = upload(sp.work[part], items, w->stream)) || (rc = upload(sp.edges[part], edges, w->stream)) ||
+        (rc = upload(sp.blocks[part], blocks, w->stream)))
+      return rc;
+    SAGE_HIP(hipStreamSynchronize(w->stream));
+  }
+  sp.tA = plan.tA;
+  sp.scatterA = plan.scatterA;
+  return SAGE_OK;
+}
+
 static int window_plan_photo_runs(SageWindow *w, int tpb, int flush)
 {
   WorkList wp;
@@ -134,7 +177,9 @@
       (rc = upload(w->photo_rec.count, wp.rec_count, w->stream)))
     return rc;
   SAGE_HIP(hipStreamSynchronize(w->stream));
-  return ph.part.reserve(std::max<size_t>(1, std::max(ph.n_work, w->photo_rec.n)) * photo_partial_floats(w->cfg.CS) * sizeof(float));
+  if ((rc = ph.part.reserve(std::max<size_t>(1, std::max(ph.n_work, w->photo_rec.n)) * photo_partial_floats(w->cfg.CS) * sizeof(float))))
+    return rc;
+  return w->solver ? window_plan_split(w) : SAGE_OK;
 }
 
 static std::vector<int> edge_tiles(const std::vector<int> &Nedge)
@@ -503,6 +548,8 @@
     return rc;
   if (w->solver && window_has_holds(w) && (rc = solver_set_holds(w->solver, w->hold, w->stream)))
     return rc;
+  if ((rc = window_plan_split(w)))
+    return rc;
   if (!fs.domain_solve)
     return SAGE_OK;
   const std::vector<int32_t> lk = window_link_pairs(w);
diff --git a/sage_slam_amd/csrc/window_eval.hip b/sage_slam_amd/csrc/window_eval.hip
--- a/sage_slam_amd/csrc/window_eval.hip
+++ b/sage_slam_amd/csrc/window_eval.hip
@@ -170,6 +170,7 @@
   PhotoFinalizeParams ph;
   GeoFinalizeParams ge;
   int n_p, n_g;
+  const int32_t *edges;
 };
 
 template <int CS>
@@ -179,10 +180,13 @@
                                                                                     : geo_finalize_lds_doubles(CS);
   __shared__ double s[LDS];
   const int bid = (int)blockIdx.x;
-  if (bid < prm.n_g)
-    geo_finalize_body<CS>(prm.ge, bid, s);
+  const bool geo = bid < prm.n_g;
+  const int slot = geo ? bid : bid - prm.n_g;
+  const int edge = prm.edges ? prm.edges[slot] : slot;
+  if (geo)
+    geo_finalize_body<CS>(prm.ge, edge, s);
   else
-    photo_finalize_body<CS>(prm.ph, bid - prm.n_g, s);
+    photo_finalize_body<CS>(prm.ph, edge, s);
 }
 
 template <bool KP>
@@ -328,6 +332,44 @@
   return ap;
 }
 
+static hipError_t launch_window_finalize(SageWindow *w, int set, const LaunchCommon &lcp, const LaunchCommon &lcg, bool merge,
+                                         const int32_t *edges, int n)
+{
+  const SageWindowConfig &c = w->cfg;
+  WindowFinalizeParams fp{};
+  fp.n_p = c.use_photo ? n : 0;
+  fp.n_g = c.use_geo ? n : 0;
+  fp.edges = edges;
+  finalize_side<PhotoEdge>(fp.ph, w->dense[kPhoto], set, lcp);
+  fp.ph.wsum = photo_weight_sum(c);
+  finalize_side<GeoEdge>(fp.ge, w->dense[kGeo], set, lcg);
+  fp.ge.weight = c.geo_weight;
+  if (merge)
+  {
+    fp.ge.photo_partials = lcp.partials;
+    fp.ge.photo_rec_first = lcp.edge_first;
+    fp.ge.photo_rec_count = lcp.edge_tiles;
+  }
+  if (c.CS == 32)
+    hipLaunchKernelGGL((window_finalize_kernel<32>), dim3(fp.n_p + fp.n_g), dim3(kFinalizeBlock), 0, w->stream, fp);
+  else
+    hipLaunchKernelGGL((window_finalize_kernel<16>), dim3(fp.n_p + fp.n_g), dim3(kFinalizeBlock), 0, w->stream, fp);
+  return hipGetLastError();
+}
+
+static hipError_t launch_window_assemble(SageWindow *w, double *packed, const int32_t *blocks, int nblocks)
+{
+  AssembleParams ap = window_assemble_params(w);
+  ap.packed = packed;
+  ap.split = 4;
+  ap.blocks = blocks;
+  if (ap.terms.stats)
+    hipLaunchKernelGGL(assemble_kernel<true>, dim3(nblocks * ap.split), dim3(512), 0, w->stream, ap);
+  else
+    hipLaunchKernelGGL(assemble_kernel<false>, dim3(nblocks * ap.split), dim3(512), 0, w->stream, ap);
+  return hipGetLastError();
+}
+
 int window_linearize_set(SageWindow *w, int set, double *dst, bool local_blocks, bool merge)
 {
   if (!w || !w->finalized)
@@ -365,48 +407,81 @@
   if (const int rct = window_launch_terms(w, set, true))
     return rct;
   if (dense)
-  {
-    WindowFinalizeParams fp{};
-    fp.n_p = c.use_photo ? w->n_edges : 0;
-    fp.n_g = c.use_geo ? w->n_edges : 0;
-    finalize_side<PhotoEdge>(fp.ph, w->dense[kPhoto], set, lcp);
-    fp.ph.wsum = photo_weight_sum(c);
-    finalize_side<GeoEdge>(fp.ge, w->dense[kGeo], set, lcg);
-    fp.ge.weight = c.geo_weight;
-    if (merge)
-    {
-      fp.ge.photo_partials = lcp.partials;
-      fp.ge.photo_rec_first = lcp.edge_first;
-      fp.ge.photo_rec_count = lcp.edge_tiles;
-    }
-    if (c.CS == 32)
-      hipLaunchKernelGGL((window_finalize_kernel<32>), dim3(fp.n_p + fp.n_g), dim3(kFinalizeBlock), 0, w->stream, fp);
-    else
-      hipLaunchKernelGGL((window_finalize_kernel<16>), dim3(fp.n_p + fp.n_g), dim3(kFinalizeBlock), 0, w->stream, fp);
-    SAGE_HIP(hipGetLastError());
-  }
-  AssembleParams ap = window_assemble_params(w);
-  if (dst)
-    ap.packed = dst;
-  ap.split = 4;
-  int nblocks = w->K + ap.nlinks + 1;
+    SAGE_HIP(launch_window_finalize(w, set, lcp, lcg, merge, nullptr, w->n_edges));
+  int nblocks = w->K + (int)w->links.size() + 1;
+  const int32_t *blocks = nullptr;
   if (local_blocks && w->dist.n_asm_blocks > 0)
   {
-    ap.blocks = w->dist.asm_blocks.as<int32_t>();
+    blocks = w->dist.asm_blocks.as<int32_t>();
     nblocks = w->dist.n_asm_blocks;
   }
-  if (ap.terms.stats)
-    hipLaunchKernelGGL(assemble_kernel<true>, dim3(nblocks * ap.split), dim3(512), 0, w->stream, ap);
-  else
-    hipLaunchKernelGGL(assemble_kernel<false>, dim3(nblocks * ap.split), dim3(512), 0, w->stream, ap);
-  SAGE_HIP(hipGetLastError());
+  double *const packed = dst ? dst : w->packed.as<double>();
+  SAGE_HIP(launch_window_assemble(w, packed, blocks, nblocks));
   window_phase_mark(w, 1);
-  if (ap.packed == w->packed.as<double>())
+  if (packed == w->packed.as<double>())
   {
     w->have_lin = true;
     w->lin_epoch = set == 0 ? w->vars_epoch : 0;
     w->spec_err_valid = false;
     w->dist.packed_reduced = false;
+  }
+  return SAGE_OK;
+}
+
+bool window_split_applies(const SageWindow *w)
+{
+  return w->split.tA > 0 && w->solver && w->world == 1 && !w->dist.allreduce && w->cfg.use_photo && w->photo_rec.flush > 0 &&
+         w->terms.kp_added.empty() && w->terms.gt_added.empty() && w->n_edges == 2 * (int)w->links.size();
+}
+
+extern "C" int sage_window_split_rows(const SageWindow *w)
+{
+  return !w ? SAGE_E_INVALID : (w->finalized && window_split_applies(w) ? w->split.tA : 0);
+}
+
+int window_linearize_part(SageWindow *w, int part)
+{
+  if (!w || !w->finalized || part < 0 || part > 1 || !window_split_applies(w))
+    return SAGE_E_STATE;
+  const SageWindowConfig &c = w->cfg;
+  const LinearizeSplit &sp = w->split;
+  const int H = (int)c.pyr.cam[0].h, W = (int)c.pyr.cam[0].w;
+  const bool merge = w->merge_ok;
+  LaunchCommon lcg = window_lc(w, kGeo), lcp = window_lc(w, kPhoto, true);
+  lcg.stage = 1;
+  lcp.stage = 1;
+  lcg.merge_geo_weight = lcp.merge_geo_weight = merge ? c.geo_weight : 0.f;
+  if (part == 0)
+  {
+    w->have_lin = false;
+    const bool have_depth = w->dpt_set == 0;
+    SAGE_HIP(launch_depth_batch(w->stream, c.CS, w->depth_items[0].as<DepthItem>(), w->n_depth, H, W, !have_depth,
+                                !(have_depth && w->dgrad_valid)));
+    w->dpt_set = 0;
+    w->dgrad_valid = true;
+    if (c.use_geo)
+    {
+      prof_attach(w, 1, lcg);
+      SAGE_HIP(launch_geo_linearize(w->stream, c.CS, nullptr, w->dense[kGeo].tab[0].as<GeoEdge>(), lcg, c.pyr.cam[0], c.eps,
+                                    c.geo_loss_param, c.geo_weight, w->dense[kGeo].out()));
+    }
+  }
+  LaunchCommon lcw = lcp;
+  lcw.work = sp.work[part].as<WorkItem>();
+  lcw.n_work = sp.n_work[part];
+  prof_attach(w, 0, lcw, part == 1);
+  SAGE_HIP(launch_photo_linearize(w->stream, c.CS, c.FS, nullptr, w->dense[kPhoto].tab[0].as<PhotoEdge>(), lcw, c.pyr,
+                                  c.photo_weights, c.eps, w->dense[kPhoto].out()));
+  SAGE_HIP(launch_window_finalize(w, 0, lcp, lcg, merge, sp.edges[part].as<int32_t>(), sp.n_edges[part]));
+  SAGE_HIP(launch_window_assemble(w, w->packed.as<double>(), sp.blocks[part].as<int32_t>(), sp.n_blocks[part]));
+  if (part == 1)
+  {
+    window_phase_mark(w, 1);
+    w->have_lin = true;
+    w->lin_epoch = w->vars_epoch;
+    w->spec_err_valid = false;
+    w->dist.packed_reduced = false;
+    window_phase_mark(w, 2);
   }
   return SAGE_OK;
 }
diff --git a/sage_slam_amd/csrc/window_lm.hip b/sage_slam_amd/csrc/window_lm.hip
--- a/sage_slam_amd/csrc/window_lm.hip
+++ b/sage_slam_amd/csrc/window_lm.hip
@@ -136,11 +136,11 @@
   return SAGE_OK;
 }
 
-static int lm_evaluate(LmSeq seq, SageWindow *w, SageLmState *st, bool first, LmEval &ev)
+static int lm_evaluate(LmSeq seq, SageWindow *w, SageLmState *st, bool first, LmEval &ev, bool with_linearize)
 {
   if (seq == LmSeq::schur)
     return evaluate_schur(w, st, first);
-  const int rc = sage_window_solve(w, st->damp, nullptr);
+  const int rc = with_linearize ? window_linearize_solve(w, st->damp) : sage_window_solve(w, st->damp, nullptr);
   if (rc == SAGE_E_NOT_PSD)
   {
     st->candidate_error = INFINITY;
@@ -180,14 +180,15 @@
   if (st->iters == 0 && st->damp <= 0)
     st->damp = cfg->init_damp;
   window_phase_mark(w, 0);
-  int rc = lm_prepare(seq, w, st);
+  const bool split = seq == LmSeq::classic && window_split_applies(w);
+  int rc = split ? SAGE_OK : lm_prepare(seq, w, st);
   if (rc)
     return rc;
   st->accepted = 0;
   for (int evals = 1;; ++evals)
   {
     LmEval ev{};
-    if ((rc = lm_evaluate(seq, w, st, evals == 1, ev)))
+    if ((rc = lm_evaluate(seq, w, st, evals == 1, ev, split && evals == 1)))
       return rc;
     if (st->candidate_error < st->error)
     {
diff --git a/sage_slam_amd/csrc/window_profile.hip b/sage_slam_amd/csrc/window_profile.hip
--- a/sage_slam_amd/csrc/window_profile.hip
+++ b/sage_slam_amd/csrc/window_profile.hip
@@ -33,7 +33,7 @@
     pf.ev_free.push_back(e);
 }
 
-void prof_attach(SageWindow *w, int which, LaunchCommon &lc)
+void prof_attach(SageWindow *w, int which, LaunchCommon &lc, bool joined)
 {
   WindowProfiler &pf = w->prof;
   if (!pf.profiling || (pf.prof_level == 2 && which != 0))
@@ -49,6 +49,7 @@
   lc.ev_start = a;
   lc.ev_stop = b;
   pf.pending[which].emplace_back(a, b);
+  pf.joined[which].push_back(joined ? 1 : 0);
 }
 
 void window_phase_mark(SageWindow *w, int which)
@@ -148,18 +149,20 @@
     return SAGE_E_INVALID;
   WindowProfiler &pf = w->prof;
   SAGE_HIP(hipStreamSynchronize(w->stream));
-  for (auto &pr : pf.pending[which])
+  for (size_t i = 0; i < pf.pending[which].size(); ++i)
   {
+    const auto &pr = pf.pending[which][i];
     float ms = 0.f;
     if (hipEventElapsedTime(&ms, pr.first, pr.second) == hipSuccess)
     {
       pf.prof_ms[which] += ms;
-      pf.prof_n[which] += 1;
+      pf.prof_n[which] += pf.joined[which][i] ? 0 : 1;
     }
     ev_put(pf, pr.first);
     ev_put(pf, pr.second);
   }
   pf.pending[which].clear();
+  pf.joined[which].clear();
   if (total_ms)
     *total_ms = pf.prof_ms[which];
   if (launches)
diff --git a/sage_slam_amd/csrc/window_solve.hip b/sage_slam_amd/csrc/window_solve.hip
--- a/sage_slam_amd/csrc/window_solve.hip
+++ b/sage_slam_amd/csrc/window_solve.hip
@@ -182,6 +182,23 @@
   return rcu;
 }
 
+int window_linearize_solve(SageWindow *w, double damp)
+{
+  if (!w || !w->finalized || !window_split_applies(w))
+    return SAGE_E_STATE;
+  int rc = window_sync_candidate(w);
+  if (rc && rc != SAGE_E_NOT_PSD)
+    return rc;
+  rc = solver_run_parts(w->solver, w->stream, w->packed.as<double>(), w->vars[0].as<float>(), w->vars[1].as<float>(), w->cfg.CS,
+                        damp, window_solve_priors(w), w->split.scatterA,
+                        [](void *user, int part) { return window_linearize_part(static_cast<SageWindow *>(user), part); }, w);
+  if (rc)
+    return rc;
+  window_phase_mark(w, 3);
+  w->cand_pending = true;
+  return SAGE_OK;
+}
+
 int window_schur_solve(SageWindow *w, double damp, double *lin_error)
 {
   const int K = w->K, B = w->B;
diff --git a/sage_slam_amd/csrc/window_state.h b/sage_slam_amd/csrc/window_state.h
--- a/sage_slam_amd/csrc/window_state.h
+++ b/sage_slam_amd/csrc/window_state.h
@@ -108,6 +108,15 @@
   int flush = 0, n = 0;
 };
 
+struct LinearizeSplit
+{
+  int tA = 0;
+  int scatterA = 0;
+  DevBuf work[2];
+  DevBuf edges[2], blocks[2];
+  int n_work[2] = {0, 0}, n_edges[2] = {0, 0}, n_blocks[2] = {0, 0};
+};
+
 struct TotalsMirror
 {
   enum : int { kTail = 0, kError = 4, kErrorTickets = 8, kMirrorTickets = 12, kDoubles = 16 };
@@ -175,6 +184,7 @@
   bool profiling = false;
   int prof_level = 0;
   std::vector<std::pair<hipEvent_t, hipEvent_t>> pending[8];
+  std::vector<char> joined[8];
   std::vector<hipEvent_t> ev_free;
   double prof_ms[8] = {0, 0, 0, 0, 0, 0, 0, 0};
   int prof_n[8] = {0, 0, 0, 0, 0, 0, 0, 0};
```
